# SimFlowCFD/RapidCFD-dev

Measured on AMD Instinct MI355X. Metric: PCG iterations/s + HBM GB/s on 10M-cell lduMatrix at 1/2/4/8 MI355X, higher is better.
Workload: dtype f64

## Files before the change

### __graft_entry__.py

```python
from __future__ import annotations

import importlib.util
import os
import subprocess
import sys

ROOT = os.path.dirname(os.path.abspath(__file__))
PKG_DIR = os.path.join(ROOT, "rapidcfd-dev_amd")
PKG_NAME = "rapidcfd_dev_amd"
HIPCC_FLAGS = ["--offload-arch=gfx950", "-O3", "-std=c++17", "-ffp-contract=off", "-fPIC", "-shared", "-pthread"]


def load_package():
    if PKG_NAME in sys.modules:
        return sys.modules[PKG_NAME]
    spec = importlib.util.spec_from_file_location(
        PKG_NAME, os.path.join(PKG_DIR, "__init__.py"), submodule_search_locations=[PKG_DIR])
    mod = importlib.util.module_from_spec(spec)
    sys.modules[PKG_NAME] = mod
    spec.loader.exec_module(mod)
    return mod


def _stale(target, sources):
    if not os.path.exists(target):
        return True
    t = os.path.getmtime(target)
    return any(os.path.getmtime(s) > t for s in sources)


def build() -> None:
    csrc = os.path.join(PKG_DIR, "csrc")
    srcs = [os.path.join(csrc, f) for f in ("engine.hip", "tiling.cpp", "gamg.cpp")]
    deps = srcs + [os.path.join(csrc, f) for f in ("kernels.hip.hpp", "tiling.hpp", "host_parallel.hpp", "gamg.hpp", "gamg_engine.inc", "assembly.inc", "limited_grad.inc", "comm.inc", "peer.inc", "multi.inc", "multi_pipe.inc", "persist.inc", "pcg_fused.inc", "host_tables.hpp", "host_match.hpp", "switches.hpp")] + [os.path.join(ROOT, "include", "mi_ldu.h")]
    so = os.path.join(PKG_DIR, "librapidcfd_amd.so")
    if _stale(so, deps):
        hipcc = os.environ.get("HIPCC", "/opt/rocm/bin/hipcc")
        subprocess.check_call([hipcc, *HIPCC_FLAGS, *srcs, "-o", so])
    foam = os.path.join(PKG_DIR, "foam")
    hipcc = os.environ.get("HIPCC", "/opt/rocm/bin/hipcc")
    libfoam = os.path.join(PKG_DIR, "libmiFoam.so")
    if _stale(libfoam, [os.path.join(foam, f) for f in ("miFoam.C", "miFoam.H", "polyMesh.C", "polyMesh.H", "solution.C", "solution.H")] + [so]):
        subprocess.check_call([hipcc, "--offload-arch=gfx950", "-O2", "-std=c++17", "-fPIC", "-shared", "-x", "hip",
                               os.path.join(foam, "miFoam.C"), os.path.join(foam, "polyMesh.C"), os.path.join(foam, "solution.C"), "-o", libfoam, "-L" + PKG_DIR,
                               "-lrapidcfd_amd", "-Wl,-rpath,$ORIGIN"])
    for name in ("pEqnFoam", "pEqnFoamPar", "polyMeshFoam", "polyMeshFoamPar", "icoFoam", "scalarTransportFoam"):
        app = os.path.join(PKG_DIR, name)
        if _stale(app, [os.path.join(foam, name + ".C"), libfoam]):
            subprocess.check_call(["g++", "-O2", "-std=c++17", os.path.join(foam, name + ".C"), "-o", app, "-L" + PKG_DIR,
                                   "-lmiFoam", "-lrapidcfd_amd", "-Wl,-rpath,$ORIGIN"])
    demo = os.path.join(ROOT, "examples", "c_abi_demo")
    if _stale(demo, [demo + ".c", so, os.path.join(ROOT, "include", "mi_ldu.h")]):
        subprocess.check_call(["gcc", "-std=c99", "-O2", "-Wall", "-Wextra", demo + ".c", "-I" + os.path.join(ROOT, "include"), "-I/opt/rocm/include",
                               "-D__HIP_PLATFORM_AMD__", "-L" + PKG_DIR, "-lrapidcfd_amd", "-L/opt/rocm/lib", "-lamdhip64",
                               "-Wl,-rpath,$ORIGIN/../rapidcfd-dev_amd", "-Wl,-rpath,/opt/rocm/lib", "-o", demo])
    sys.path.insert(0, ROOT)
    from oracle import oracle as _oracle
    _oracle.build()
    if os.path.isdir("/root/reference"):
        subprocess.check_call(["make", "-s", "-C", os.path.join(ROOT, "oracle"), "dropin"])
    pkg = load_package()
    pkg.engine.lib()


def smoke() -> None:
    import numpy as np
    import torch

    build()
    pkg = load_package()
    from oracle import oracle as orc
    eng = pkg.engine
    assert torch.cuda.is_available(), "smoke() needs a GPU"
    dev = torch.device("cuda:0")
    case = pkg.synthetic.box_case(24, 20, 16)
    ctx = eng.Context(0, torch.cuda.current_stream().cuda_stream)
    addr = eng.Addressing(ctx, case.n_cells, case.lower_addr, case.upper_addr)
    mat = eng.Matrix(addr)
    t = lambda a: torch.from_numpy(np.ascontiguousarray(a)).to(dev)
    mat.set_coeffs(t(case.diag), t(case.upper), None)
    psi = torch.zeros(case.n_cells, dtype=torch.float64, device=dev)
    perf = mat.pcg(psi, t(case.source), "diagonal", tolerance=1e-8, maxIter=500)
    ref_psi, ref = orc.System([case]).pcg(np.zeros(case.n_cells), case.source, "diagonal", tolerance=1e-8, maxIter=500)
    assert perf["nIterations"] == ref["nIterations"], (perf["nIterations"], ref["nIterations"])
    h, hr = perf["history"], ref["history"]
    rel = np.max(np.abs(h - hr)) / hr[0]
    assert rel < 1e-10, rel
    err = np.max(np.abs(psi.cpu().numpy() - ref_psi)) / np.max(np.abs(ref_psi))
    assert err < 1e-10, err
    print(f"smoke ok: PCG {perf['nIterations']} iterations, residual history rel diff {rel:.2e}, psi rel diff {err:.2e}")


if __name__ == "__main__":
    build()
    print("build ok")
```

### include/mi_ldu.h

```cpp
#ifndef MI_LDU_H
#define MI_LDU_H

#include <stdint.h>

#ifdef __cplusplus
extern "C" {
#endif

typedef struct mi_ctx_s *mi_ctx_t;
typedef struct mi_addr_s *mi_addr_t;
typedef struct mi_matrix_s *mi_matrix_t;
typedef struct mi_gamg_s *mi_gamg_t;
typedef struct mi_patch_s *mi_patch_t;
typedef struct mi_comm_s *mi_comm_t;

enum {
    MI_OK = 0,
    MI_ERR_ARG = -1,
    MI_ERR_DEVICE = -2,
    MI_ERR_ALLOC = -3,
    MI_ERR_STATE = -4,
    MI_ERR_LIMIT = -5,
    MI_ERR_UNSUPPORTED = -6
};

enum { MI_PRECOND_NONE = 0, MI_PRECOND_DIAGONAL = 1, MI_PRECOND_AINV = 2 };

typedef struct {
    double initialResidual;
    double finalResidual;
    double normFactor;
    int32_t nIterations;
    int32_t converged;
    int32_t singular;
    int32_t reserved;
} mi_solver_perf;

typedef struct {
    double tolerance;
    double relTol;
    int32_t maxIter;
    int32_t minIter;
} mi_solver_controls;

int mi_ctx_create(int device, void *hip_stream, mi_ctx_t *out);
int mi_ctx_destroy(mi_ctx_t ctx);
int mi_ctx_synchronize(mi_ctx_t ctx);
int mi_ctx_set_option(mi_ctx_t ctx, const char *name, int32_t value);
#define MI_STAT_PERSIST_PCG 0
#define MI_STAT_PERSIST_DPCG 1
#define MI_STAT_BARRIER_LITMUS 2
#define MI_STAT_GAMG_GRAPH_ATTACHED 3
#define MI_STAT_PCG_FUSED_RP 4
#define MI_STAT_PCG_GRAPH 5
#define MI_STAT_PBICG_MULTI 6
#define MI_STAT_PBICG_DEVICE 7
#define MI_STAT_PBICG_HOST_STEPPED 8
#define MI_STAT_PBICGSTAB_DEVICE 9
#define MI_STAT_PBICGSTAB_HOST_STEPPED 10
#define MI_STAT_PBICGSTAB_MID_EXIT 11
int mi_ctx_stat(mi_ctx_t ctx, int32_t which, int64_t *out);
const char *mi_last_error(void);
int mi_device_available(void);

int mi_addr_create(mi_ctx_t ctx, int32_t n_cells, int32_t n_faces,
                   const int32_t *lower_addr_host, const int32_t *upper_addr_host,
                   int32_t n_patches, const int32_t *patch_sizes,
                   const int32_t *const *patch_face_cells_host, mi_addr_t *out);
int mi_addr_create_coupled(mi_ctx_t ctx, int32_t n_cells, int32_t n_faces,
                           const int32_t *lower_addr_host, const int32_t *upper_addr_host,
                           int32_t n_patches, const int32_t *patch_sizes,
                           const int32_t *const *patch_face_cells_host,
                           const int32_t *const *patch_nbr_cells_host, mi_addr_t *out);
int mi_addr_set_ami_patch(mi_addr_t addr, int32_t patch, int32_t nbr_patch, const int32_t *start_host_or_null,
                          const int32_t *address_host_or_null, const double *weights_host_or_null,
                          const uint8_t *low_weight_host_or_null);
int mi_addr_set_ami_patch_remote(mi_addr_t addr, int32_t patch, int32_t transport_patch, int32_t n_partner_faces,
                                 const int32_t *start_host, const int32_t *address_host, const double *weights_host,
                                 const uint8_t *low_weight_host_or_null);
int mi_addr_set_ami_patch_remote_multi(mi_addr_t addr, int32_t patch, int32_t n_transports, const int32_t *transport_patches_host,
                                       const int32_t *n_partner_faces_host, const int32_t *start_host, const int32_t *address_host,
                                       const double *weights_host, const uint8_t *low_weight_host_or_null);
int mi_addr_set_ami_face_areas(mi_addr_t addr, int32_t patch, const double *mag_sf_host);
int mi_addr_create_ordered(mi_ctx_t ctx, int32_t n_cells, int32_t n_faces, const int32_t *lower_host, const int32_t *upper_host,
                           int32_t n_patches, const int32_t *patch_sizes, const int32_t *const *patch_face_cells_host,
                           const int32_t *const *patch_nbr_cells_host_or_null, int32_t n_tiles, const int32_t *tile_cell_start_host_or_null,
                           mi_addr_t *out);
int mi_addr_create_adopted(mi_ctx_t ctx, int32_t n_cells, int32_t n_faces, const int32_t *lower_host, const int32_t *upper_host,
                           int32_t n_patches, const int32_t *patch_sizes, const int32_t *const *patch_face_cells_host,
                           const int32_t *const *patch_nbr_cells_host_or_null, int32_t *cell_new_to_old_out, int32_t *face_new_to_old_out,
                           uint8_t *face_flipped_out, int32_t *lower_out, int32_t *upper_out, mi_addr_t *out);
int mi_layout_adopt_host(int32_t n_cells, int32_t n_faces, const int32_t *lower_host, const int32_t *upper_host, int32_t n_patches,
                         const int32_t *patch_sizes, const int32_t *const *patch_face_cells_host, const int32_t *const *patch_nbr_cells_host_or_null,
                         int32_t *cell_new_to_old_out, int32_t *face_new_to_old_out, uint8_t *face_flipped_out, int32_t *lower_out,
                         int32_t *upper_out, int32_t *n_tiles_out);
int mi_addr_tile_starts(mi_addr_t addr, int32_t *tile_cell_start_out_host);
int mi_addr_is_ordered(mi_addr_t addr);
int mi_addr_destroy(mi_addr_t addr);
int32_t mi_addr_n_cells(mi_addr_t addr);
int32_t mi_addr_n_faces(mi_addr_t addr);
int32_t mi_addr_n_tiles(mi_addr_t addr);
int32_t mi_addr_n_ext(mi_addr_t addr);
int mi_addr_cell_perm(mi_addr_t addr, int32_t *engine_to_caller_host);
int mi_addr_stats(mi_addr_t addr, int64_t stats[8]);

int mi_matrix_create(mi_addr_t addr, mi_matrix_t *out);
mi_addr_t mi_matrix_addr(mi_matrix_t m);
int mi_matrix_destroy(mi_matrix_t m);
int mi_matrix_set_coeffs(mi_matrix_t m, const double *diag_dev, const double *upper_dev,
                         const double *lower_dev);
int mi_matrix_set_interface_coeffs(mi_matrix_t m, int32_t patch, const double *bou_coeffs_dev,
                                   const double *int_coeffs_dev);
int mi_matrix_set_patch_transform(mi_matrix_t m, int32_t patch, double factor);

int mi_halo_pack_engine(mi_addr_t addr, const double *x_engine_dev, double *send_dev);
int mi_addr_patch_offsets(mi_addr_t addr, int32_t *offsets_host );

int mi_vec_to_engine(mi_addr_t addr, const double *x_caller_dev, double *x_engine_dev);
int mi_vec_from_engine(mi_addr_t addr, const double *x_engine_dev, double *x_caller_dev);

int mi_amul(mi_matrix_t m, const double *psi_dev, double *Apsi_dev);
int mi_tmul(mi_matrix_t m, const double *psi_dev, double *Tpsi_dev);
int mi_sumA(mi_matrix_t m, double *sumA_dev);
int mi_residual(mi_matrix_t m, const double *psi_dev, const double *source_dev, double *rA_dev);
int mi_H(mi_matrix_t m, const double *psi_dev, double *H_dev);
int mi_H1(mi_matrix_t m, double *H1_dev);
int mi_faceH(mi_matrix_t m, const double *psi_dev, double *faceH_dev);
int mi_matrix_set_ext(mi_matrix_t m, const double *ext_values_dev);

int mi_amul_engine(mi_matrix_t m, const double *psi_e, double *Apsi_e, int which);
int mi_tmul_engine(mi_matrix_t m, const double *psi_e, double *Tpsi_e, int which);

int mi_precondition_engine(mi_matrix_t m, int kind, int transpose, const double *rA_e, double *wA_e);
int mi_residual_engine(mi_matrix_t m, const double *psi_e, const double *source_e, double *rA_e);
int mi_jacobi_smooth_engine(mi_matrix_t m, double omega, double *psi_e, const double *source_e, int32_t n_sweeps);
int mi_norm_factor_engine(mi_matrix_t m, const double *psi_e, const double *source_e, const double *Apsi_e, double *out_host);

int mi_precondition(mi_matrix_t m, int kind, int transpose, const double *rA_dev, double *wA_dev);

int mi_jacobi_smooth(mi_matrix_t m, double omega, double *psi_dev, const double *source_dev,
                     int32_t n_sweeps);

int mi_sum(mi_ctx_t ctx, const double *a_dev, int64_t n, double *out_host);
int mi_sum_prod(mi_ctx_t ctx, const double *a_dev, const double *b_dev, int64_t n, double *out_host);
int mi_sum_mag(mi_ctx_t ctx, const double *a_dev, int64_t n, double *out_host);
int mi_norm_factor(mi_matrix_t m, const double *psi_dev, const double *source_dev,
                   const double *Apsi_dev, double *out_host);

int mi_pcg_solve(mi_matrix_t m, double *psi_dev, const double *source_dev,
                 const mi_solver_controls *controls, int precond,
                 mi_solver_perf *perf_out, double *residual_history_host, int32_t history_len);
int mi_pcg_begin(mi_matrix_t m, const double *psi0_dev, const double *source_dev,
                 const mi_solver_controls *controls, int precond, int32_t history_len);
int mi_pcg_iterate(mi_matrix_t m, int32_t n_iters, float *amul_ms_sum);
int mi_pcg_iterate_sampled(mi_matrix_t m, int32_t n_iters, int32_t event_stride, float *amul_ms_sum);
int mi_pcg_end(mi_matrix_t m, double *psi_out_dev, mi_solver_perf *perf_out,
               double *residual_history_host, int32_t history_len);

typedef struct {
    double tolerance, relTol;
    int32_t maxIter, minIter;
    int32_t nPreSweeps, preSweepsLevelMultiplier, maxPreSweeps;
    int32_t nPostSweeps, postSweepsLevelMultiplier, maxPostSweeps;
    int32_t nFinestSweeps, scaleCorrection;
    double omega;
    int32_t directSolveCoarsest;
    int32_t reserved;
} mi_gamg_controls;
int mi_gamg_create(mi_addr_t fine_addr, const double *face_weights_host, int32_t n_cells_in_coarsest_level,
                   int32_t merge_levels, int forward_init, mi_gamg_t *out);
int mi_gamg_create_dummy(mi_addr_t fine_addr, int32_t n_levels, mi_gamg_t *out);
int mi_gamg_create_coupled(mi_addr_t fine_addr, const double *face_weights_host,
                           int32_t n_cells_in_coarsest_level, int32_t merge_levels, int forward_init, mi_comm_t reduce_or_null,
                           mi_comm_t halo_or_null, const int32_t *patch_rank,
                           const int32_t *patch_nbr_patch_or_null, mi_gamg_t *out);
int mi_gamg_destroy(mi_gamg_t g);
int32_t mi_gamg_n_levels(mi_gamg_t g);
int mi_gamg_forward_out(mi_gamg_t g);
int mi_gamg_level_sizes(mi_gamg_t g, int32_t level, int32_t out4[4]);
int mi_gamg_solve(mi_gamg_t g, mi_matrix_t m, double *psi_dev, const double *source_dev,
                  const mi_gamg_controls *controls, mi_solver_perf *perf_out,
                  double *residual_history_host, int32_t history_len);
int mi_gamg_restrict(mi_gamg_t g, int32_t level, const double *fine_dev, double *coarse_dev);
int mi_gamg_prolong(mi_gamg_t g, int32_t level, const double *coarse_dev, double *fine_dev);
int mi_gamg_update(mi_gamg_t g, mi_matrix_t m);
int mi_gamg_level_matrix(mi_gamg_t g, int32_t level, mi_matrix_t *level_matrix_out);
int mi_gamg_scale(mi_matrix_t m, double *field_dev, double *Acf_dev, const double *source_dev);
int mi_gamg_solve_coarsest(mi_gamg_t g, const double *source_dev, double *corr_dev);
int mi_gamg_level_coeffs(mi_gamg_t g, mi_matrix_t m, int32_t level, double *diag_out_dev,
                         double *upper_out_dev, double *lower_out_dev);

int mi_row_face_op(mi_addr_t addr, int kind, const double *lower_dev, const double *upper_dev, double *inout_dev);
int mi_fvm_laplacian(mi_addr_t addr, const double *delta_coeffs_dev, const double *gamma_magsf_dev,
                     double *upper_out_dev, double *diag_out_dev);
int mi_fvm_div(mi_addr_t addr, const double *weights_dev, const double *face_flux_dev,
               double *lower_out_dev, double *upper_out_dev, double *diag_out_dev);
int mi_surface_integrate(mi_addr_t addr, const double *ssf_dev, const double *vol_dev_or_null, double *ivf_dev);
int mi_face_interpolate(mi_addr_t addr, const double *lambda_dev, const double *phi_dev, double *sf_dev);
int mi_fvm_ddt_euler(mi_ctx_t ctx, int64_t n, double r_delta_t, double rho, const double *vol_dev,
                     const double *psi_old_dev, double *diag_out_dev, double *source_out_dev);
int mi_upwind_weights(mi_ctx_t ctx, int64_t n_faces, const double *face_flux_dev, double *weights_out_dev);
int mi_limited_linear_weights(mi_addr_t addr, double k, const double *cd_weights_dev, const double *face_flux_dev,
                              const double *phi_dev, const double *gradx_dev, const double *grady_dev,
                              const double *gradz_dev, const double *cx_dev, const double *cy_dev,
                              const double *cz_dev, double *weights_out_dev, double *limiter_out_dev_or_null);
enum { MI_LIM_LIMITED_LINEAR, MI_LIM_VAN_LEER, MI_LIM_MUSCL, MI_LIM_MINMOD, MI_LIM_SUPERBEE, MI_LIM_UMIST,
       MI_LIM_VAN_ALBADA, MI_LIM_OSPRE, MI_LIM_QUICK, MI_LIM_LIMITED_CUBIC, MI_LIM_GAMMA, MI_LIM_SFCD };
typedef struct mi_limiter {
    int32_t kind;
    int32_t vector_form;
    int32_t bounded;
    double k, lower, upper;
} mi_limiter;
// ... 193 lines not shown
```

### rapidcfd-dev_amd/csrc/engine.hip

```cpp
#include <hip/hip_ext.h>
#include "../../include/mi_ldu.h"
#include "kernels.hip.hpp"
#include "tiling.hpp"
#include "host_parallel.hpp"
#include "switches.hpp"

#include <algorithm>
#include <atomic>
#include <cstdio>
#include <cstdlib>
#include <cstring>
#include <condition_variable>
#include <functional>
#include <map>
#include <set>
#include <mutex>
#include <string>
#include <thread>
#include <vector>

using namespace mi;
constexpr int HALO_NV = 6;

namespace {

thread_local std::string g_err;
int fail(int code, const std::string& msg) { g_err = msg; return code; }

#define HIPCHK(expr)                                                                          \
    do {                                                                                      \
        hipError_t e__ = (expr);                                                              \
        if (e__ != hipSuccess)                                                                \
            return fail(MI_ERR_DEVICE, std::string(#expr) + ": " + hipGetErrorString(e__));   \
    } while (0)
#define MICHK(expr) do { int r__ = (expr); if (r__ != MI_OK) return r__; } while (0)

template <class T>
struct DevBuf {
    T* p = nullptr;
    size_t n = 0;
    DevBuf() = default;
    DevBuf(const DevBuf&) = delete;
    DevBuf& operator=(const DevBuf&) = delete;
    ~DevBuf() { release(); }
    void release() { if (p) { (void)hipFree(p); p = nullptr; n = 0; } }
    int alloc(size_t count)
    {
        if (count == n && p) return MI_OK;
        release();
        if (hipMalloc((void**)&p, (count ? count : 1) * sizeof(T)) != hipSuccess) { p = nullptr; return fail(MI_ERR_ALLOC, "hipMalloc failed"); }
        n = count;
        return MI_OK;
    }
    template <class A>
    int upload(const std::vector<T, A>& v, hipStream_t s)
    {
        MICHK(alloc(v.size()));
        if (!v.empty()) HIPCHK(hipMemcpyAsync(p, v.data(), v.size() * sizeof(T), hipMemcpyHostToDevice, s));
        return MI_OK;
    }
};

}

struct mi_ctx_s {
    int device = 0;
    hipStream_t stream = nullptr;
    bool ownStream = false;
    DevBuf<double> partial;
    DevBuf<double> scalars;
    DevBuf<PcgState> state;
    PcgState* hostState = nullptr;
    double* hostScal = nullptr;
    hipEvent_t ev0 = nullptr, ev1 = nullptr;
    hipStream_t sideStream = nullptr;
    hipEvent_t evSideGo = nullptr, evSideDone = nullptr;
    int nCU = 0;
    bool keepSlotTables = false;
    int tileFlags = 0, attachEvents = 0, persist = 0, xcdRows = 0, deferPsi = 0, fusePerm = 0, pairAT = 0, fusePrologue = 0, multiPipe = 0, winDirect = 0, gamgGraphAttached = 0;
    int pcgPersist = 0, pcgFuseRP = 0, pcgFuseTest = 0, persistGrid = 0, persistShared = 0, fuseFinal = 0, amulBS = 0, pcgBatch = 0, pcgGraph = 0, pbicgHostStepped = 0;
    int gamgDeviceInvert = 0, gamgAlwaysAgglomerate = 0, gamgGraph = 0, gamgFuse = 0;
    int64_t stats[12] = {};
    int persistCoop = -1;
    uint64_t faultEpoch = 0;
    struct mi_matrix_s* session = nullptr;
    std::set<const void*> ldsAttrSet;
    std::map<std::pair<const void*, size_t>, int> occCache;
};

struct CtxSwitch { Switch id; int mi_ctx_s::*member; };
static constexpr CtxSwitch CTX_SWITCHES[] = {
    {SW_TILE_FLAGS, &mi_ctx_s::tileFlags}, {SW_EVENT_ATTACH, &mi_ctx_s::attachEvents}, {SW_TILE_PERSIST, &mi_ctx_s::persist}, {SW_XCD_ROWS, &mi_ctx_s::xcdRows},
    {SW_PCG_DEFER_PSI, &mi_ctx_s::deferPsi}, {SW_FUSE_PERM, &mi_ctx_s::fusePerm}, {SW_PBICG_PAIR, &mi_ctx_s::pairAT}, {SW_FUSE_PROLOGUE, &mi_ctx_s::fusePrologue},
    {SW_MULTI_PIPE, &mi_ctx_s::multiPipe}, {SW_WIN_DIRECT, &mi_ctx_s::winDirect}, {SW_GAMG_GRAPH_ATTACHED, &mi_ctx_s::gamgGraphAttached}, {SW_PCG_PERSIST, &mi_ctx_s::pcgPersist},
    {SW_PCG_FUSE_RP, &mi_ctx_s::pcgFuseRP}, {SW_PCG_FUSE_TEST, &mi_ctx_s::pcgFuseTest}, {SW_PERSIST_GRID, &mi_ctx_s::persistGrid}, {SW_PERSIST_SHARED, &mi_ctx_s::persistShared},
    {SW_PCG_FUSE_FINAL, &mi_ctx_s::fuseFinal}, {SW_AMUL_BS, &mi_ctx_s::amulBS}, {SW_PCG_BATCH, &mi_ctx_s::pcgBatch}, {SW_PCG_GRAPH, &mi_ctx_s::pcgGraph},
    {SW_PBICG_HOST_STEPPED, &mi_ctx_s::pbicgHostStepped}, {SW_GAMG_DEVICE_INVERT, &mi_ctx_s::gamgDeviceInvert}, {SW_GAMG_ALWAYS_AGGLOMERATE, &mi_ctx_s::gamgAlwaysAgglomerate},
    {SW_GAMG_GRAPH, &mi_ctx_s::gamgGraph}, {SW_GAMG_FUSE, &mi_ctx_s::gamgFuse},
};
constexpr bool ctx_switches_match_table()
{
    for (int s = 0; s < SW_COUNT; ++s) {
        int n = 0;
        for (const CtxSwitch& e : CTX_SWITCHES) n += e.id == s;
        if (n != ((sw::table[s].when & sw::CTX) ? 1 : 0)) return false;
    }
    return true;
}
static_assert(ctx_switches_match_table(), "CTX_SWITCHES: exactly one entry for every sw::CTX row of switches.hpp");
static void ctx_store(mi_ctx_s* c, const CtxSwitch& s, int value) { c->*s.member = s.id == SW_PCG_FUSE_RP ? (value != 0 ? -1 : 0) : value; }

struct mi_addr_s {
    mi_ctx_s* ctx = nullptr;
    TileLayout L;
    DevBuf<int32_t> e2c, c2e, tileCellStart, tileSlotStart, tileIfaceSlot0, tileHaloStart, haloCell, tileSliceStart, sliceEntryStart;
    DevBuf<uint32_t> entries, entries16;
    DevBuf<int32_t> sliceEntryStart16, tileSbStart;
    DevBuf<uint16_t> slotBase;
    bool compact = false;
    DevBuf<int32_t> slotFace, extSlot, interiorTiles, boundaryTiles, patchFaceCellsE, faceSlot, lowerAddr, upperAddr;
    DevBuf<int32_t> ownerStartC, losortStartC, losortC;
    DevBuf<uint32_t> row16; DevBuf<uint16_t> losort16; DevBuf<int32_t> rowEsc, rowEscStart;
    struct RowPlan { bool tiles = false; int bs = 256, blocks = 0, maxFaces = 0, capForced = 0; } rowPlan[2];
    DevBuf<double> relaxD0, relaxSumOff;
    DevBuf<uint8_t> setMask; DevBuf<double> setVal;
    Table<int32_t> lowerHost, upperHost;
    int32_t nInterior = 0, nBoundary = 0, nLocalPatches = 0;
    Table<char> patchIsLocal;
    DevBuf<int32_t> ifaceNbrCaller;
    DevBuf<int32_t> haloSrc;
    Table<Table<int32_t>> patchFaceCellsHost, patchNbrCellsHost;
    int64_t nEntries = 0, nHaloTot = 0;
    struct AmiPatch {
        int32_t patch = 0, nbrPatch = 0, n = 0, extOff = 0;
        Table<int32_t> transports, partCount;
        int32_t transport = -1, nPartner = 0;
        DevBuf<int32_t> start, cellE, ownE; DevBuf<double> w; bool hasLow = false;
        Table<int32_t> hStart, hAddr; Table<double> hW, hMagSf;
    };
    Table<AmiPatch*> ami;
    bool amiRemote = false;
    ~mi_addr_s() { for (AmiPatch* q : ami) delete q; }
    bool identity = false;
    const int32_t* perm() const { return identity ? nullptr : e2c.p; }
};

struct mi_dpcg_s { double *psi = nullptr, *src = nullptr, *pA = nullptr, *wA = nullptr, *rA = nullptr, *scal = nullptr, *send = nullptr; int precond = 0; };

enum WorkVec : size_t {
    WV_OP_X = 0, WV_OP_Y = 1, WV_OP_B = 2,
    WV_NF_APSI = 0, WV_NF_SUMA = 1, WV_NF_SRC = 2, WV_NF_PSI = 3,
    WV_PSI = 3, WV_SRC = 4, WV_PA = 5, WV_WA = 6, WV_RA = 7,
    WV_PT = 8, WV_WT = 9, WV_RT = 10,
    WV_STAB_YA = 6, WV_STAB_AYA = 8, WV_STAB_SA = 9, WV_STAB_ZA = 10, WV_STAB_TA = 11, WV_STAB_RA0 = 12,
    WV_STAB_RES1 = 13,
    WV_SMOOTH_PSI2 = 8, WV_BENCH_ZERO = 14, WV_MULTI = 16, WV_MULTI_STRIDE = 11
};

struct mi_matrix_s {
    mi_addr_s* addr = nullptr;
    mi_dpcg_s dp;
    DevBuf<double> diagE, upE, lowE, rD, sumAE;
    bool asym = false, bound = false, rDValid = false, sumAValid = false;
    Table<double> patchFactor;
    uint64_t epoch = 0;
    Table<DevBuf<double>*> work;
    DevBuf<double> hist, tilePartial;
    DevBuf<PcgState> mstate; DevBuf<double> mpartial, mhist, mtilePartial; PcgState* mhostState = nullptr;
    DevBuf<double> persistScratch;
    uint64_t persistFaultEpoch = 0;
    DevBuf<double> persistZ;
    int histLen = 0;
    int pcgIt = 0, pcgPrecond = MI_PRECOND_DIAGONAL;
    bool pcgActive = false;
    bool pcgPReady = false;
    DevBuf<unsigned int> fusedBar;
    unsigned int fusedGen = 0;
    Table<hipEvent_t> evPool;
    hipGraphExec_t pcgGraph = nullptr;
    struct { int precond = -1, batch = 0, histLen = 0; const void* hist = nullptr; const void* psi = nullptr; } pcgGraphKey;
    bool gateDone = false;
    double *proY2 = nullptr, *proY3 = nullptr;
    const double *callerX = nullptr, *callerB = nullptr; double* callerY = nullptr;
    hipEvent_t kevStart = nullptr, kevStop = nullptr;
    struct mi_dpcg_comm_s* dpc = nullptr;
    DevBuf<double> sendBuf, dscal;
    ~mi_matrix_s();
    int vec(size_t k, double** out)
    {
        while (work.size() <= k) work.push_back(new DevBuf<double>());
        const size_t need = (size_t)addr->L.nCells + (size_t)addr->L.nExt;
        if (work[k]->n != need) {
            MICHK(work[k]->alloc(need));
            HIPCHK(hipMemsetAsync(work[k]->p, 0, need * sizeof(double), addr->ctx->stream));
        }
        *out = work[k]->p;
        return MI_OK;
    }
    struct Slot { size_t k; double** out; };
    int vecs(std::initializer_list<Slot> slots) { for (const Slot& v : slots) MICHK(vec(v.k, v.out)); return MI_OK; }
};

static int solver_entry(const char* fn, const mi_matrix_s* m, bool args_ok, bool check_session = true)
{
    if (!m || !args_ok) return fail(MI_ERR_ARG, std::string(fn) + ": bad argument");
    if (!m->bound) return fail(MI_ERR_STATE, "matrix coefficients not bound");
    if (check_session && m->addr->ctx->session) return fail(MI_ERR_STATE, std::string(fn) + ": a PCG session (mi_pcg_begin) is active on this context; call mi_pcg_end first");
    return MI_OK;
}

bool comm_remote(const mi_matrix_s* m);
bool comm_attached(const mi_matrix_s* m);
bool comm_any_ami(const mi_matrix_s* m);
bool comm_any_factor(const mi_matrix_s* m);
bool comm_any_compact(const mi_matrix_s* m);
bool matrix_has_factor(const mi_matrix_s* m);
void comm_inherit_factor_flag(mi_matrix_s* level, const mi_matrix_s* fine);
int64_t comm_n_global(const mi_matrix_s* m);
int comm_exchange_start(mi_matrix_s* m, const double* send, double* vec);
int comm_exchange_wait(mi_matrix_s* m);
int comm_allreduce(mi_matrix_s* m, double* dev, size_t n);
bool peer_halo_ready(const mi_matrix_s* m);
int peer_exchange_push(mi_matrix_s* m, const double* x);
int peer_exchange_pull(mi_matrix_s* m, double* x);
int peer_exchange_push_n(mi_matrix_s* m, int nv, const double* const* xs);
int peer_exchange_pull_n(mi_matrix_s* m, int nv, double* const* xs);
bool peer_win_direct(mi_matrix_s* m);
int peer_check(mi_matrix_s* m);
int dpcg_flush_if_fused(mi_matrix_s* m);
bool peer_reduce_ready(const mi_matrix_s* m);
int peer_globalize(mi_matrix_s* m, int n, double* const* P);
int pcg_solve_attached(mi_matrix_s* m, double* psi_io, const double* source, const mi_solver_controls* ctl, int precond,
                       mi_solver_perf* perf, double* hist_host, int32_t hist_len);

extern "C" const char* mi_last_error(void) { return g_err.c_str(); }

extern "C" int mi_device_available(void)
{
    int n = 0;
    if (hipGetDeviceCount(&n) != hipSuccess || n <= 0) return 0;
    hipDeviceProp_t prop;
    if (hipGetDeviceProperties(&prop, 0) != hipSuccess) return 0;
    return strncmp(prop.gcnArchName, "gfx950", 6) == 0 ? 1 : 0;
}

extern "C" int mi_ctx_create(int device, void* hip_stream, mi_ctx_t* out)
{
    if (!out) return fail(MI_ERR_ARG, "out is NULL");
    int n = 0;
    const hipError_t e0 = hipGetDeviceCount(&n);
    if (e0 != hipSuccess || n <= 0)
        return fail(MI_ERR_DEVICE, std::string("no HIP device visible: the engine has no CPU fallback (hipGetDeviceCount: ") + hipGetErrorString(e0) + ", " + std::to_string(n) + " devices)");
    if (device < 0 || device >= n) return fail(MI_ERR_ARG, "device index out of range");
    HIPCHK(hipSetDevice(device));
    hipDeviceProp_t prop;
    HIPCHK(hipGetDeviceProperties(&prop, device));
    if (strncmp(prop.gcnArchName, "gfx950", 6) != 0)
        return fail(MI_ERR_DEVICE, std::string("engine is built for gfx950 only, found ") + prop.gcnArchName);
    mi_ctx_s* c = new mi_ctx_s();
    c->device = device;
    if (hip_stream) c->stream = (hipStream_t)hip_stream;
    else { if (hipStreamCreate(&c->stream) != hipSuccess) { delete c; return fail(MI_ERR_DEVICE, "hipStreamCreate failed"); } c->ownStream = true; }
    int r = c->partial.alloc(4 * RG);
    if (r == MI_OK) r = c->scalars.alloc(16);
    if (r == MI_OK) r = c->state.alloc(1);
    if (r != MI_OK) { delete c; return r; }
    if (hipHostMalloc((void**)&c->hostState, sizeof(PcgState)) != hipSuccess ||
        hipHostMalloc((void**)&c->hostScal, 16 * sizeof(double)) != hipSuccess ||
        hipEventCreate(&c->ev0) != hipSuccess || hipEventCreate(&c->ev1) != hipSuccess) {
        delete c; return fail(MI_ERR_DEVICE, "pinned host / event allocation failed");
    }
    { hipDeviceProp_t pr; if (hipGetDeviceProperties(&pr, device) == hipSuccess) c->nCU = pr.multiProcessorCount; }
    for (const CtxSwitch& s : CTX_SWITCHES) ctx_store(c, s, sw::get(s.id));
    if (c->pcgBatch < 1) c->pcgBatch = 1;
    if (c->amulBS != 256 && c->amulBS != 512 && c->amulBS != 1024) c->amulBS = 0;
    *out = c;
    return MI_OK;
}

extern "C" int mi_ctx_destroy(mi_ctx_t c)
{
    if (!c) return MI_OK;
    (void)hipSetDevice(c->device);
    (void)hipStreamSynchronize(c->stream);
    if (c->hostState) (void)hipHostFree(c->hostState);
    if (c->hostScal) (void)hipHostFree(c->hostScal);
    if (c->ev0) (void)hipEventDestroy(c->ev0);
    if (c->ev1) (void)hipEventDestroy(c->ev1);
    if (c->sideStream) { (void)hipStreamSynchronize(c->sideStream); (void)hipStreamDestroy(c->sideStream); }
    if (c->evSideGo) (void)hipEventDestroy(c->evSideGo);
    if (c->evSideDone) (void)hipEventDestroy(c->evSideDone);
    if (c->ownStream) (void)hipStreamDestroy(c->stream);
    delete c;
    return MI_OK;
}

extern "C" int mi_ctx_synchronize(mi_ctx_t c)
{
    if (!c) return fail(MI_ERR_ARG, "ctx is NULL");
    HIPCHK(hipStreamSynchronize(c->stream));
    return MI_OK;
}

extern "C" int mi_ctx_set_option(mi_ctx_t c, const char* name, int32_t value)
{
    if (!c || !name) return fail(MI_ERR_ARG, "mi_ctx_set_option: bad argument");
    for (const CtxSwitch& s : CTX_SWITCHES)
        if (sw::table[s.id].option && strcmp(name, sw::table[s.id].option) == 0) { ctx_store(c, s, value); return MI_OK; }
    return fail(MI_ERR_ARG, "mi_ctx_set_option: unknown option");
}

extern "C" int mi_ctx_stat(mi_ctx_t c, int32_t which, int64_t* out)
{
    if (!c || !out || which < 0 || which >= (int32_t)(sizeof(c->stats) / sizeof(c->stats[0]))) return fail(MI_ERR_ARG, "mi_ctx_stat: bad argument");
    *out = c->stats[which];
    return MI_OK;
}

static int32_t tile_reorder() { return sw::get(SW_TILE_REORDER); }
static TileParams addr_tile_params(mi_ctx_t ctx, int32_t n_cells, bool coarse, bool ordered, int32_t n_tiles, const int32_t* tile_cell_start)
{
    TileParams prm;
    prm.tileCells = sw::get(SW_TILE_CELLS);
    if (prm.tileCells <= 0) {
        int target = 1024;
        if (coarse && sw::get(SW_SMALL_TILES)) target = (int)(((int64_t)n_cells / std::max(1, ctx->nCU) + 63) / 64 * 64);
        prm.tileCells = std::min(1024, std::max(128, target));
    }
    prm.slotCap = sw::get(SW_TILE_SLOTS);
    prm.reorder = tile_reorder();
// ... 284 lines not shown
    if (r != MI_OK) { delete q; return r; }
    HIPCHK(hipStreamSynchronize(s));
    a->ami.push_back(q);
    a->patchIsLocal[(size_t)patch] = 2;
    a->nLocalPatches++;
    a->amiRemote = true;
    return MI_OK;
}
extern "C" int mi_addr_set_ami_patch_remote_multi(mi_addr_t a, int32_t patch, int32_t n_transports, const int32_t* transport_patches, const int32_t* n_partner_faces,
                                                  const int32_t* start, const int32_t* address, const double* weights, const uint8_t* low_weight)
{
    if (!a || patch < 0 || patch >= a->L.nPatches || n_transports < 1 || !transport_patches || !n_partner_faces || !start || !address || !weights)
        return fail(MI_ERR_ARG, "mi_addr_set_ami_patch_remote_multi: bad argument");
    const int32_t n = (int32_t)a->patchFaceCellsHost[(size_t)patch].size();
    Table<int32_t> tr(transport_patches, transport_patches + n_transports), cnt(n_partner_faces, n_partner_faces + n_transports), off((size_t)n_transports + 1, 0);
    for (int32_t q = 0; q < n_transports; ++q) { if (cnt[(size_t)q] < 0) return fail(MI_ERR_ARG, "mi_addr_set_ami_patch_remote_multi: negative partner face count"); off[(size_t)q + 1] = off[(size_t)q] + cnt[(size_t)q]; }
    for (int32_t i = 0; i < n; ++i) if (start[i + 1] < start[i]) return fail(MI_ERR_ARG, "mi_addr_set_ami_patch_remote_multi: start must be non-decreasing");
    const int32_t na = n > 0 || start ? start[n] : 0;
    Table<int32_t> slot((size_t)na), face((size_t)na);
    for (int32_t k = 0; k < na; ++k) {
        if (address[k] < 0 || address[k] >= off[(size_t)n_transports]) return fail(MI_ERR_ARG, "mi_addr_set_ami_patch_remote_multi: address outside the partner pieces");
        int32_t q = 0;
        while (address[k] >= off[(size_t)q + 1]) ++q;
        slot[(size_t)k] = q; face[(size_t)k] = address[k] - off[(size_t)q];
    }
    return ami_remote_impl(a, patch, tr, cnt, start, slot.data(), face.data(), address, weights, low_weight);
}
extern "C" int mi_addr_set_ami_patch_remote(mi_addr_t a, int32_t patch, int32_t transport_patch, int32_t n_partner_faces, const int32_t* start,
                                            const int32_t* address, const double* weights, const uint8_t* low_weight)
{
    return mi_addr_set_ami_patch_remote_multi(a, patch, 1, &transport_patch, &n_partner_faces, start, address, weights, low_weight);
}

extern "C" int mi_addr_set_ami_face_areas(mi_addr_t a, int32_t patch, const double* mag_sf)
{
    if (!a || !mag_sf) return fail(MI_ERR_ARG, "mi_addr_set_ami_face_areas: bad argument");
    for (mi_addr_s::AmiPatch* q : a->ami) if (q->patch == patch) { q->hMagSf.assign(mag_sf, mag_sf + q->n); return MI_OK; }
    return fail(MI_ERR_ARG, "mi_addr_set_ami_face_areas: not a cyclicAMI patch");
}

extern "C" int mi_matrix_set_patch_transform(mi_matrix_t m, int32_t patch, double factor)
{
    if (!m || patch < 0 || patch >= m->addr->L.nPatches) return fail(MI_ERR_ARG, "mi_matrix_set_patch_transform: bad argument");
    if (m->addr->patchIsLocal[(size_t)patch] == 1 && factor != 1.0)
        return fail(MI_ERR_UNSUPPORTED, "mi_matrix_set_patch_transform: a transformed cyclic patch is declared through mi_addr_set_ami_patch (one-to-one, unit weights)");
    if (comm_attached(m) && factor != 1.0 && !comm_any_factor(m))
        return fail(MI_ERR_STATE, "mi_matrix_set_patch_transform: the first transformed patch of a decomposed case is declared BEFORE mi_matrix_attach_comm (the ranks agree on the solver pipeline there)");
    if (m->patchFactor.empty()) m->patchFactor.assign((size_t)m->addr->L.nPatches, 1.0);
    if (m->patchFactor[(size_t)patch] != factor) ++m->epoch;
    m->patchFactor[(size_t)patch] = factor;
    return MI_OK;
}
extern "C" int32_t mi_addr_n_cells(mi_addr_t a) { return a ? a->L.nCells : 0; }
extern "C" int32_t mi_addr_n_faces(mi_addr_t a) { return a ? a->L.nFaces : 0; }
extern "C" int32_t mi_addr_n_tiles(mi_addr_t a) { return a ? a->L.nTiles : 0; }
extern "C" int32_t mi_addr_n_ext(mi_addr_t a) { return a ? a->L.nExt : 0; }

extern "C" int mi_addr_cell_perm(mi_addr_t a, int32_t* e2c_host)
{
    if (!a || !e2c_host) return fail(MI_ERR_ARG, "mi_addr_cell_perm: bad argument");
    memcpy(e2c_host, a->L.e2c.data(), sizeof(int32_t) * (size_t)a->L.nCells);
    return MI_OK;
}

extern "C" int mi_addr_patch_offsets(mi_addr_t a, int32_t* off)
{
    if (!a || !off) return fail(MI_ERR_ARG, "mi_addr_patch_offsets: bad argument");
    memcpy(off, a->L.patchOffset.data(), sizeof(int32_t) * a->L.patchOffset.size());
    return MI_OK;
}

static size_t lds_bytes(const TileLayout& L, bool asym, bool ainv, int32_t* offLow, int32_t* offX, int32_t* offRD, int32_t* offSB = nullptr)
{
    const int32_t slots = (L.maxSlots + 3) & ~1;
    const int32_t xlen = ((L.maxCells + 63) & ~63) + L.maxHalo + 2;
    int32_t off = slots;
    *offLow = off; if (asym) off += slots;
    *offX = off; off += (xlen + 1) & ~1;
    *offRD = off; if (ainv) off += (xlen + 1) & ~1;
    if (offSB) { *offSB = off; if (L.compact) off += (L.maxCells + L.maxHalo + 1 + 3) / 4 + 1; }
    return (size_t)off * sizeof(double);
}

extern "C" int mi_addr_stats(mi_addr_t a, int64_t st[8])
{
    if (!a || !st) return fail(MI_ERR_ARG, "mi_addr_stats: bad argument");
    int32_t o1, o2, o3;
    st[0] = a->L.nTiles; st[1] = a->L.totalSlots; st[2] = a->nEntries; st[3] = a->nHaloTot;
    st[4] = a->L.maxCells; st[5] = a->L.maxSlots; st[6] = a->L.maxHalo;
    int32_t o4;
    st[7] = (int64_t)lds_bytes(a->L, false, false, &o1, &o2, &o3, &o4);
    return MI_OK;
}

static uint64_t next_epoch() { static std::atomic<uint64_t> e{0}; return ++e; }
extern "C" mi_addr_t mi_matrix_addr(mi_matrix_t m) { return m ? m->addr : nullptr; }
extern "C" int mi_matrix_create(mi_addr_t a, mi_matrix_t* out)
{
    if (!a || !out) return fail(MI_ERR_ARG, "mi_matrix_create: bad argument");
    HIPCHK(hipSetDevice(a->ctx->device));
    mi_matrix_s* m = new mi_matrix_s();
    m->addr = a;
    int r = m->diagE.alloc((size_t)a->L.nCells);
    if (r == MI_OK) r = m->upE.alloc((size_t)a->L.totalSlots);
    if (r != MI_OK) { delete m; return r; }
    if (hipMemsetAsync(m->upE.p, 0, sizeof(double) * (size_t)a->L.totalSlots, a->ctx->stream) != hipSuccess) { delete m; return fail(MI_ERR_DEVICE, "memset failed"); }
    *out = m;
    return MI_OK;
}

extern "C" int mi_matrix_destroy(mi_matrix_t m)
{
    if (m) { (void)hipSetDevice(m->addr->ctx->device); (void)hipStreamSynchronize(m->addr->ctx->stream); delete m; }
    return MI_OK;
}

extern "C" int mi_matrix_set_coeffs(mi_matrix_t m, const double* diag, const double* upper, const double* lower)
{
    if (!m || !diag || (!upper && m->addr->L.nFaces > 0)) return fail(MI_ERR_ARG, "mi_matrix_set_coeffs: bad argument");
    mi_addr_s* a = m->addr;
    hipStream_t s = a->ctx->stream;
    HIPCHK(hipSetDevice(a->ctx->device));
    const bool asym = (lower != nullptr);
    if (asym && m->lowE.n != (size_t)a->L.totalSlots) {
        MICHK(m->lowE.alloc((size_t)a->L.totalSlots));
        HIPCHK(hipMemcpyAsync(m->lowE.p, m->upE.p, sizeof(double) * (size_t)a->L.totalSlots, hipMemcpyDeviceToDevice, s));
    }
    m->asym = asym;
    k_gather_perm<<<RG, RB, 0, s>>>(diag, a->perm(), m->diagE.p, a->L.nCells);
    k_fill_slots<<<2048, 256, 0, s>>>(upper, lower, a->slotFace.p, m->upE.p, asym ? m->lowE.p : nullptr, a->L.totalSlots);
    HIPCHK(hipGetLastError());
    m->bound = true;
    m->rDValid = false; m->sumAValid = false;
    m->epoch = next_epoch();
    return MI_OK;
}

extern "C" int mi_matrix_set_interface_coeffs(mi_matrix_t m, int32_t patch, const double* bou, const double* inte)
{
    if (!m || !bou || patch < 0 || patch >= m->addr->L.nPatches) return fail(MI_ERR_ARG, "mi_matrix_set_interface_coeffs: bad argument");
    mi_addr_s* a = m->addr;
    HIPCHK(hipSetDevice(a->ctx->device));
    const int32_t off = a->L.patchOffset[patch], n = a->L.patchOffset[(size_t)patch + 1] - off;
    if (n == 0) return MI_OK;
    k_fill_iface<<<(n + 255) / 256, 256, 0, a->ctx->stream>>>(bou, inte, a->extSlot.p + off, m->upE.p, m->asym ? m->lowE.p : nullptr, n);
    HIPCHK(hipGetLastError());
    m->sumAValid = false;
    m->epoch = next_epoch();
    return MI_OK;
}

namespace {

template <int OP, bool ASYM, bool TRANS, bool C16>
int launch_tile_bs(mi_matrix_s* m, const TileArgs& args, int nTiles, size_t lds)
{
    hipStream_t s = m->addr->ctx->stream;
    int bs = m->addr->ctx->amulBS;
    if (bs == 0) bs = (lds > 53 * 1024) ? 1024 : (m->addr->L.maxCells <= 256 ? 256 : 512);
    if (nTiles <= 0) return MI_OK;
#define MI_LAUNCH(BS)                                                                                                   \
    {                                                                                                                   \
        mi_ctx_s* cx = m->addr->ctx;                                                                                    \
        const void* fn = (const void*)tile_kernel<OP, ASYM, TRANS, BS, C16>;                                            \
        if (!cx->ldsAttrSet.count(fn)) {           \
            HIPCHK(hipFuncSetAttribute(fn, hipFuncAttributeMaxDynamicSharedMemorySize, 159 * 1024));                    \
            cx->ldsAttrSet.insert(fn);                                                                                  \
        }                                                                                                               \
        int grid = nTiles;                                                                                              \
        if (cx->persist) {                                                                                              \
            int& occ = cx->occCache[std::make_pair(fn, lds)];                                                           \
            if (occ == 0) {                                                                                             \
                int nb = 0;                                                                                             \
                HIPCHK(hipOccupancyMaxActiveBlocksPerMultiprocessor(&nb, fn, BS, lds));                                 \
                occ = nb > 0 ? nb : 1;                                                                                  \
            }                                                                                                           \
            const int slots = ((occ * cx->nCU * cx->persist) / 8) * 8;                                                  \
            if (slots >= 8 && nTiles > 2 * slots) grid = slots;                                                         \
        }                                                                                                               \
        if (m->kevStart)            \
            hipExtLaunchKernelGGL((tile_kernel<OP, ASYM, TRANS, BS, C16>), dim3(grid), dim3(BS), (uint32_t)lds, s, m->kevStart, m->kevStop, 0, args); \
        else                                                                                                            \
        tile_kernel<OP, ASYM, TRANS, BS, C16><<<grid, BS, lds, s>>>(args);                                                   \
    }
    if (bs == 1024) MI_LAUNCH(1024)
    else if (bs == 512) MI_LAUNCH(512)
    else MI_LAUNCH(256)
#undef MI_LAUNCH
    HIPCHK(hipGetLastError());
    return MI_OK;
}

template <int OP>
int launch_tile_win(mi_matrix_s* m, bool trans, const double* x, const double* b, const double* rD, double* y,
                    double omega, double* dotPartial, double* dotPartial2);

template <int OP>
int launch_tile(mi_matrix_s* m, bool trans, const double* x, const double* b, const double* rD, double* y,
                double omega, int which, double* dotPartial = nullptr, double* dotPartial2 = nullptr)
{
    mi_addr_s* a = m->addr;
    if (!m->bound) return fail(MI_ERR_STATE, "matrix coefficients not bound (mi_matrix_set_coeffs)");
    TileArgs t;
    t.tileCellStart = a->tileCellStart.p; t.tileSlotStart = a->tileSlotStart.p; t.tileIfaceSlot0 = a->tileIfaceSlot0.p; t.tileHaloStart = a->tileHaloStart.p;
    t.haloCell = a->haloCell.p; t.tileSliceStart = a->tileSliceStart.p; t.sliceEntryStart = a->sliceEntryStart.p;
    t.entries = a->entries.p; t.entries16 = a->entries16.p; t.sliceEntryStart16 = a->sliceEntryStart16.p; t.slotBase = reinterpret_cast<const uint32_t*>(a->slotBase.p); t.tileSbStart = a->tileSbStart.p;
    t.diag = m->diagE.p; t.up = m->upE.p; t.low = m->lowE.p;
    t.x = x; t.b = b; t.rD = rD; t.y = y; t.omega = omega; t.dotPartial = dotPartial; t.dotPartial2 = dotPartial2; t.flags = a->ctx->tileFlags;
    if (OP == OP_PROLOGUE) { t.y2 = m->proY2; t.y3 = m->proY3; }

    const size_t lds = lds_bytes(a->L, m->asym, OP == OP_AINV, &t.offLow, &t.offX, &t.offRD, &t.offSB);
    if (lds > 159 * 1024) return fail(MI_ERR_LIMIT, "tile needs more than 159 KiB of LDS");
    int nTiles = a->L.nTiles;
    t.tileList = nullptr;
    if (which == 1) { t.tileList = a->interiorTiles.p; nTiles = a->nInterior; }
    else if (which == 2) { t.tileList = a->boundaryTiles.p; nTiles = a->nBoundary; }
    t.nPos = nTiles;
    t.done = m->gateDone ? &a->ctx->state.p->done : nullptr;
    if (m->callerY) {
        if constexpr (OP == OP_AMUL || OP == OP_RESIDUAL || OP == OP_H || OP == OP_SUMA || OP == OP_H1) {
            t.perm = a->e2c.p; t.haloSrc = a->haloSrc.p; t.xExt = x ? x + a->L.nCells : nullptr;
            t.x = m->callerX; t.b = m->callerB; t.y = m->callerY;
            mi_ctx_s* cx = a->ctx;
            hipStream_t s = cx->stream;
            const bool big = lds > 53 * 1024;
#define MI_LAUNCH_PERM(ASYM, TRANS)                                                                                      \
            {                                                                                                           \
                const void* fn = big ? (const void*)tile_kernel_perm<OP, ASYM, TRANS, 1024> : (const void*)tile_kernel_perm<OP, ASYM, TRANS, 512>; \
                if (!cx->ldsAttrSet.count(fn)) { HIPCHK(hipFuncSetAttribute(fn, hipFuncAttributeMaxDynamicSharedMemorySize, 159 * 1024)); cx->ldsAttrSet.insert(fn); } \
                if (big) tile_kernel_perm<OP, ASYM, TRANS, 1024><<<nTiles, 1024, lds, s>>>(t);                           \
                else tile_kernel_perm<OP, ASYM, TRANS, 512><<<nTiles, 512, lds, s>>>(t);                                 \
            }
            if (nTiles > 0) {
                if (m->asym) { if (trans) MI_LAUNCH_PERM(true, true) else MI_LAUNCH_PERM(true, false) }
                else MI_LAUNCH_PERM(false, false)
            }
#undef MI_LAUNCH_PERM
            HIPCHK(hipGetLastError());
            return MI_OK;
        } else return fail(MI_ERR_STATE, "caller-order tile launch of an operator without a caller-order form");
    }
    if (a->compact) {
        if (m->asym) {
            if (trans) return launch_tile_bs<OP, true, true, true>(m, t, nTiles, lds);
            return launch_tile_bs<OP, true, false, true>(m, t, nTiles, lds);
        }
        return launch_tile_bs<OP, false, false, true>(m, t, nTiles, lds);
    }
    if (m->asym) {
        if (trans) return launch_tile_bs<OP, true, true, false>(m, t, nTiles, lds);
        return launch_tile_bs<OP, true, false, false>(m, t, nTiles, lds);
    }
    return launch_tile_bs<OP, false, false, false>(m, t, nTiles, lds);
}

struct FxArgs {
    const int32_t* map = nullptr; const double* coarse = nullptr; double* out = nullptr;
    const double *field = nullptr, *acf = nullptr, *src = nullptr, *scal = nullptr, *add = nullptr;
    unsigned int* foldCounter = nullptr; double* foldOut = nullptr;
};
inline bool tile_fx_usable(const mi_matrix_s* m) { return m->bound && !m->addr->compact && m->addr->L.nExt == 0 && m->addr->ami.empty() && !m->callerY && !m->gateDone; }
template <int OP, int XMODE>
int launch_tile_fx(mi_matrix_s* m, const FxArgs& fx, const double* b, double* y, double omega, double* dotPartial = nullptr, double* dotPartial2 = nullptr)
{
    mi_addr_s* a = m->addr;
    if (!tile_fx_usable(m)) return fail(MI_ERR_STATE, "launch_tile_fx: matrix not eligible");
    TileArgs t;
    t.tileCellStart = a->tileCellStart.p; t.tileSlotStart = a->tileSlotStart.p; t.tileIfaceSlot0 = a->tileIfaceSlot0.p; t.tileHaloStart = a->tileHaloStart.p;
    t.haloCell = a->haloCell.p; t.tileSliceStart = a->tileSliceStart.p; t.sliceEntryStart = a->sliceEntryStart.p;
    t.entries = a->entries.p; t.entries16 = nullptr; t.sliceEntryStart16 = nullptr; t.slotBase = nullptr; t.tileSbStart = nullptr;
    t.diag = m->diagE.p; t.up = m->upE.p; t.low = m->lowE.p;
    t.x = nullptr; t.b = b; t.rD = nullptr; t.y = y; t.omega = omega; t.dotPartial = dotPartial; t.dotPartial2 = dotPartial2; t.flags = a->ctx->tileFlags;
    t.fxMap = fx.map; t.fxCoarse = fx.coarse; t.fxOut = fx.out; t.fxField = fx.field; t.fxAcf = fx.acf; t.fxSrc = fx.src; t.fxScal = fx.scal; t.fxAdd = fx.add;
    t.foldCounter = fx.foldCounter; t.foldOut = fx.foldOut;
    size_t lds = lds_bytes(a->L, m->asym, false, &t.offLow, &t.offX, &t.offRD, &t.offSB);
    if (lds > 159 * 1024) return fail(MI_ERR_LIMIT, "tile needs more than 159 KiB of LDS");
    if (fx.foldOut) lds = std::max(lds, (size_t)(2 * RG + 2 * (RB / 64) + 2) * sizeof(double));
    const int nTiles = a->L.nTiles;
    t.tileList = nullptr; t.nPos = nTiles; t.done = nullptr;
    if (nTiles <= 0) return MI_OK;
    mi_ctx_s* cx = a->ctx;
    hipStream_t s = cx->stream;
    int bs = cx->amulBS;
    if (bs == 0) bs = (lds > 53 * 1024) ? 1024 : (a->L.maxCells <= 256 ? 256 : 512);
#define MI_LAUNCH_FX(ASYM, BS)                                                                                           \
    {                                                                                                                   \
        const void* fn = (const void*)tile_kernel_fx<OP, ASYM, BS, XMODE>;                                              \
        if (!cx->ldsAttrSet.count(fn)) { HIPCHK(hipFuncSetAttribute(fn, hipFuncAttributeMaxDynamicSharedMemorySize, 159 * 1024)); cx->ldsAttrSet.insert(fn); } \
        tile_kernel_fx<OP, ASYM, BS, XMODE><<<nTiles, BS, lds, s>>>(t);                                                 \
    }
    if (m->asym) { if (bs == 1024) MI_LAUNCH_FX(true, 1024) else if (bs == 512) MI_LAUNCH_FX(true, 512) else MI_LAUNCH_FX(true, 256) }
    else { if (bs == 1024) MI_LAUNCH_FX(false, 1024) else if (bs == 512) MI_LAUNCH_FX(false, 512) else MI_LAUNCH_FX(false, 256) }
#undef MI_LAUNCH_FX
    HIPCHK(hipGetLastError());
    return MI_OK;
}

int ensure_rD(mi_matrix_s* m)
{
    if (m->rDValid) return MI_OK;
    mi_addr_s* a = m->addr;
    const size_t need = (size_t)a->L.nCells + (size_t)a->L.nExt;
    if (m->rD.n != need) {
        MICHK(m->rD.alloc(need));
        HIPCHK(hipMemsetAsync(m->rD.p, 0, need * sizeof(double), a->ctx->stream));
    }
    k_recip<<<RG, RB, 0, a->ctx->stream>>>(m->rD.p, m->diagE.p, a->L.nCells);
    HIPCHK(hipGetLastError());
    m->rDValid = true;
    return MI_OK;
}

bool aligned16(const void* p) { return (reinterpret_cast<uintptr_t>(p) & 15u) == 0; }
// ... 348 lines not shown
    MICHK(m->vec(WV_OP_Y, &scratch));
    double *cur = psi_e, *nxt = scratch;
    for (int sw = 0; sw < n_sweeps; ++sw) {
        if (a->L.nExt > 0 && sw > 0 && !comm_remote(m))
            HIPCHK(hipMemcpyAsync(cur + a->L.nCells, nxt + a->L.nCells, sizeof(double) * (size_t)a->L.nExt, hipMemcpyDeviceToDevice, s));
        MICHK(tile_op<OP_JACOBI>(m, false, cur, source_e, nullptr, nxt, omega));
        double* t = cur; cur = nxt; nxt = t;
    }
    if (cur != psi_e) HIPCHK(hipMemcpyAsync(psi_e, cur, sizeof(double) * (size_t)a->L.nCells, hipMemcpyDeviceToDevice, s));
    return MI_OK;
}

namespace {
int norm_factor_engine(mi_matrix_s* m, const double* psi_e, const double* src_e, const double* Apsi_e, double* sumA_scratch, double* out)
{
    mi_addr_s* a = m->addr;
    mi_ctx_s* c = a->ctx;
    hipStream_t s = c->stream;
    const int64_t n = a->L.nCells;
    MICHK(launch_tile<OP_SUMA>(m, false, nullptr, nullptr, nullptr, sumA_scratch, 0.0, 0));
    double sumPsi = 0;
    MICHK(reduce_sync_fwd(m, psi_e, &sumPsi));
    const double avg = sumPsi / (double)(comm_attached(m) ? comm_n_global(m) : n);
    k_normfactor<<<RG, RB, 0, s>>>(Apsi_e, src_e, sumA_scratch, avg, n, c->partial.p);
    k_reduce_final<<<1, RB, 0, s>>>(c->partial.p, c->scalars.p);
    HIPCHK(hipGetLastError());
    if (comm_attached(m)) MICHK(comm_allreduce(m, c->scalars.p, 1));
    HIPCHK(hipMemcpyAsync(c->hostScal, c->scalars.p, sizeof(double), hipMemcpyDeviceToHost, s));
    HIPCHK(hipStreamSynchronize(s));
    *out = c->hostScal[0] + SP_SMALL;
    return MI_OK;
}
}
extern "C" int mi_norm_factor(mi_matrix_t m, const double* psi, const double* source, const double* Apsi, double* out)
{
    MICHK(solver_entry("mi_norm_factor", m, psi && source && Apsi && out));
    mi_addr_s* a = m->addr;
    HIPCHK(hipSetDevice(a->ctx->device));
    hipStream_t s = a->ctx->stream;
    const int64_t n = a->L.nCells;
    double *ApsiE, *sumA, *srcE, *psiE;
    MICHK(m->vecs({{WV_NF_APSI, &ApsiE}, {WV_NF_SUMA, &sumA}, {WV_NF_SRC, &srcE}, {WV_NF_PSI, &psiE}}));
    k_gather_perm<<<RG, RB, 0, s>>>(Apsi, a->perm(), ApsiE, n);
    k_gather_perm<<<RG, RB, 0, s>>>(source, a->perm(), srcE, n);
    k_gather_perm<<<RG, RB, 0, s>>>(psi, a->perm(), psiE, n);
    return norm_factor_engine(m, psiE, srcE, ApsiE, sumA, out);
}
extern "C" int mi_norm_factor_engine(mi_matrix_t m, const double* psi_e, const double* source_e, const double* Apsi_e, double* out)
{
    MICHK(solver_entry("mi_norm_factor_engine", m, psi_e && source_e && Apsi_e && out));
    HIPCHK(hipSetDevice(m->addr->ctx->device));
    double* sumA;
    MICHK(m->vec(WV_NF_SUMA, &sumA));
    return norm_factor_engine(m, psi_e, source_e, Apsi_e, sumA, out);
}

namespace {

int precond_engine(mi_matrix_s* m, int kind, bool transpose, const double* r, double* w)
{
    mi_addr_s* a = m->addr;
    hipStream_t s = a->ctx->stream;
    const int64_t n = a->L.nCells;
    if (kind == MI_PRECOND_NONE) { HIPCHK(hipMemcpyAsync(w, r, sizeof(double) * (size_t)n, hipMemcpyDeviceToDevice, s)); return MI_OK; }
    MICHK(ensure_rD(m));
    if (kind == MI_PRECOND_DIAGONAL) { k_mul<<<RG, RB, 0, s>>>(w, m->rD.p, r, n); HIPCHK(hipGetLastError()); return MI_OK; }
    if (kind == MI_PRECOND_AINV) return launch_tile<OP_AINV>(m, transpose, r, nullptr, m->rD.p, w, 0.0, 0);
    return fail(MI_ERR_ARG, "unknown preconditioner kind");
}

template <int KIND>
int reduce_sync(mi_matrix_s* m, const double* a, const double* b, double* out)
{
    mi_ctx_s* c = m->addr->ctx;
    k_reduce<KIND><<<RG, RB, 0, c->stream>>>(a, b, (int64_t)m->addr->L.nCells, c->partial.p);
    k_reduce_final<<<1, RB, 0, c->stream>>>(c->partial.p, c->scalars.p);
    HIPCHK(hipGetLastError());
    if (comm_attached(m)) MICHK(comm_allreduce(m, c->scalars.p, 1));
    HIPCHK(hipMemcpyAsync(c->hostScal, c->scalars.p, sizeof(double), hipMemcpyDeviceToHost, c->stream));
    HIPCHK(hipStreamSynchronize(c->stream));
    if (comm_attached(m)) MICHK(peer_check(m));
    *out = c->hostScal[0];
    return MI_OK;
}

int reduce_sync_fwd(mi_matrix_s* m, const double* a, double* out) { return reduce_sync<RED_SUM>(m, a, nullptr, out); }

int solve_prologue(mi_matrix_s* m, const mi_solver_controls* ctl, const double* psi_e, const double* src_e,
                   double* wA, double* rA, int histLen)
{
    mi_addr_s* a = m->addr;
    mi_ctx_s* c = a->ctx;
    hipStream_t s = c->stream;
    const int64_t n = a->L.nCells;
    if (m->hist.n < (size_t)(histLen > 0 ? histLen : 1)) MICHK(m->hist.alloc((size_t)(histLen > 0 ? histLen : 1)));
    m->histLen = histLen;
    PcgState h;
    memset(&h, 0, sizeof(h));
    h.tolerance = ctl->tolerance; h.relTol = ctl->relTol; h.maxIter = ctl->maxIter; h.minIter = ctl->minIter;
    *c->hostState = h;
    HIPCHK(hipMemcpyAsync(c->state.p, c->hostState, sizeof(PcgState), hipMemcpyHostToDevice, s));
    if (c->fusePrologue) {
        const bool needSumA = !m->sumAValid;
        if (needSumA && m->sumAE.n != (size_t)n) MICHK(m->sumAE.alloc((size_t)n));
        m->proY2 = rA; m->proY3 = needSumA ? m->sumAE.p : nullptr;
        const int rc = tile_op<OP_PROLOGUE>(m, false, psi_e, src_e, nullptr, wA, 0.0);
        m->proY2 = nullptr; m->proY3 = nullptr;
        MICHK(rc);
        m->sumAValid = true;
        double* P = c->partial.p;
        k_reduce<RED_SUM><<<RG, RB, 0, s>>>(psi_e, nullptr, n, P + 2 * RG);
        if (comm_attached(m)) {
            k_reduce_final<<<1, RB, 0, s>>>(P + 2 * RG, c->scalars.p);
            MICHK(comm_allreduce(m, c->scalars.p, 1));
            k_normfactor_mag<true><<<RG, RB, 0, s>>>(wA, src_e, m->sumAE.p, c->scalars.p, (double)comm_n_global(m), n, P, P + RG);
            k_reduce_final2<<<2, RB, 0, s>>>(P, c->scalars.p + 1, P + RG, c->scalars.p + 2);
            MICHK(comm_allreduce(m, c->scalars.p + 1, 2));
            k_solve_init<true><<<1, RB, 0, s>>>(c->state.p, c->scalars.p + 1, c->scalars.p + 2, m->hist.p, histLen);
        } else {
            k_normfactor_mag<false><<<RG, RB, 0, s>>>(wA, src_e, m->sumAE.p, P + 2 * RG, (double)n, n, P, P + RG);
            k_solve_init<false><<<1, RB, 0, s>>>(c->state.p, P, P + RG, m->hist.p, histLen);
        }
        HIPCHK(hipGetLastError());
        return MI_OK;
    }
    MICHK(tile_op<OP_AMUL>(m, false, psi_e, nullptr, nullptr, wA, 0.0));
    k_sub<<<RG, RB, 0, s>>>(rA, src_e, wA, n);
    if (!m->sumAValid) {
        if (m->sumAE.n != (size_t)n) MICHK(m->sumAE.alloc((size_t)n));
        MICHK(launch_tile<OP_SUMA>(m, false, nullptr, nullptr, nullptr, m->sumAE.p, 0.0, 0));
        m->sumAValid = true;
    }
    double sumPsi = 0;
    MICHK(reduce_sync<RED_SUM>(m, psi_e, nullptr, &sumPsi));
    const double avg = sumPsi / (double)(comm_attached(m) ? comm_n_global(m) : n);
    k_normfactor<<<RG, RB, 0, s>>>(wA, src_e, m->sumAE.p, avg, n, c->partial.p);
    k_reduce<RED_MAG><<<RG, RB, 0, s>>>(rA, nullptr, n, c->partial.p + RG);
    if (comm_attached(m)) {
        k_reduce_final2<<<2, RB, 0, s>>>(c->partial.p, c->scalars.p + 1, c->partial.p + RG, c->scalars.p + 2);
        MICHK(comm_allreduce(m, c->scalars.p + 1, 2));
        k_solve_init<true><<<1, RB, 0, s>>>(c->state.p, c->scalars.p + 1, c->scalars.p + 2, m->hist.p, histLen);
    } else
    k_solve_init<false><<<1, RB, 0, s>>>(c->state.p, c->partial.p, c->partial.p + RG, m->hist.p, histLen);
    HIPCHK(hipGetLastError());
    return MI_OK;
}

int fetch_state(mi_ctx_s* c)
{
    HIPCHK(hipMemcpyAsync(c->hostState, c->state.p, sizeof(PcgState), hipMemcpyDeviceToHost, c->stream));
    HIPCHK(hipStreamSynchronize(c->stream));
    if (c->hostState->fault) {
        c->faultEpoch++;
        return fail(MI_ERR_DEVICE, "persistent PCG kernel: a workgroup never reached a grid barrier (ran out of polls); the results of this solve are not valid");
    }
    return MI_OK;
}

template <class State>
void fill_perf(const State& h, mi_solver_perf* p)
{
    p->initialResidual = h.initialResidual; p->finalResidual = h.finalResidual; p->normFactor = h.normFactor;
    p->nIterations = h.nIterations; p->converged = h.converged; p->singular = h.singular; p->reserved = 0;
}

int copy_hist(hipStream_t s, const double* hist_dev, int dev_len, double* hist_host, int len, int nIter, bool sync = true)
{
    if (!hist_host || len <= 0) return MI_OK;
    int cnt = nIter + 1; if (cnt > len) cnt = len; if (cnt > dev_len) cnt = dev_len;
    if (cnt > 0) {
        HIPCHK(hipMemcpyAsync(hist_host, hist_dev, sizeof(double) * (size_t)cnt, hipMemcpyDeviceToHost, s));
        if (sync) HIPCHK(hipStreamSynchronize(s));
    }
    return MI_OK;
}
int copy_hist(mi_matrix_s* m, double* hist_host, int len, int nIter) { return copy_hist(m->addr->ctx->stream, m->hist.p, m->histLen, hist_host, len, nIter); }

struct PcgVecs { double *psi, *src, *pA, *wA, *rA; };
struct BicgVecs : PcgVecs { double *pT, *wT, *rT; };
struct StabVecs { double *psi, *src, *pA, *yA, *rA, *AyA, *sA, *zA, *tA, *rA0; };
int work_vecs(mi_matrix_s* m, PcgVecs& v) { return m->vecs({{WV_PSI, &v.psi}, {WV_SRC, &v.src}, {WV_PA, &v.pA}, {WV_WA, &v.wA}, {WV_RA, &v.rA}}); }
int work_vecs(mi_matrix_s* m, BicgVecs& v) { MICHK(work_vecs(m, static_cast<PcgVecs&>(v))); return m->vecs({{WV_PT, &v.pT}, {WV_WT, &v.wT}, {WV_RT, &v.rT}}); }
int work_vecs(mi_matrix_s* m, StabVecs& v) { return m->vecs({{WV_PSI, &v.psi}, {WV_SRC, &v.src}, {WV_PA, &v.pA}, {WV_STAB_YA, &v.yA}, {WV_RA, &v.rA},
                                                             {WV_STAB_AYA, &v.AyA}, {WV_STAB_SA, &v.sA}, {WV_STAB_ZA, &v.zA}, {WV_STAB_TA, &v.tA}, {WV_STAB_RA0, &v.rA0}}); }
template <class Vecs>
int stage_in(mi_matrix_s* m, Vecs& v, const double* psi, const double* source)
{
    mi_addr_s* a = m->addr;
    MICHK(work_vecs(m, v));
    k_gather_perm<<<RG, RB, 0, a->ctx->stream>>>(psi, a->perm(), v.psi, a->L.nCells);
    k_gather_perm<<<RG, RB, 0, a->ctx->stream>>>(source, a->perm(), v.src, a->L.nCells);
    return MI_OK;
}

struct GateDone { mi_matrix_s* m; explicit GateDone(mi_matrix_s* mm) : m(mm) { m->gateDone = true; } ~GateDone() { m->gateDone = false; } };
int iter_limit(const mi_solver_controls* ctl) { return ctl->maxIter + (ctl->minIter > ctl->maxIter ? ctl->minIter : 0); }

template <class Enqueue, class Fetch, class Done>
int drive_batches(mi_matrix_s* m, const mi_solver_controls* ctl, const int& it, int first, Enqueue enqueue, Fetch fetch, Done done)
{
    const int batch = m->addr->ctx->pcgBatch, limit = iter_limit(ctl);
    int nb = batch < first ? batch : first;
    while (!done() && it <= limit) {
        MICHK(enqueue(nb));
        MICHK(fetch());
        MICHK(peer_check(m));
        nb = nb * 2 > batch ? batch : nb * 2;
    }
    return MI_OK;
}
template <class Enqueue>
int drive_batches(mi_matrix_s* m, const mi_solver_controls* ctl, const int& it, int first, Enqueue enqueue)
{
    mi_ctx_s* c = m->addr->ctx;
    return drive_batches(m, ctl, it, first, enqueue, [c] { return fetch_state(c); }, [c] { return c->hostState->done != 0; });
}

int finish_device(mi_matrix_s* m, const double* psi_e, double* psi_out, mi_solver_perf* perf, double* hist_host, int hist_len, int (*flush)(mi_matrix_s*) = nullptr)
{
    mi_addr_s* a = m->addr; mi_ctx_s* c = a->ctx;
    if (flush) MICHK(flush(m));
    k_scatter_perm<<<RG, RB, 0, c->stream>>>(psi_e, a->perm(), psi_out, a->L.nCells);
    HIPCHK(hipGetLastError());
    if (perf) fill_perf(*c->hostState, perf);
    MICHK(copy_hist(m, hist_host, hist_len, c->hostState->nIterations));
    HIPCHK(hipStreamSynchronize(c->stream));
    return MI_OK;
}

int globalize(mi_matrix_s* m, double* PA, double* PB = nullptr)
{
    if (!comm_attached(m)) return MI_OK;
    if (peer_reduce_ready(m)) { double* P[2] = {PA, PB}; return peer_globalize(m, PB ? 2 : 1, P); }
    mi_ctx_s* c = m->addr->ctx;
    hipStream_t s = c->stream;
    double* sc = c->scalars.p + 10;
    if (PB) k_reduce_final2<<<2, RB, 0, s>>>(PA, sc, PB, sc + 1);
    else k_reduce_final<<<1, RB, 0, s>>>(PA, sc);
    MICHK(comm_allreduce(m, sc, PB ? 2 : 1));
    k_spread_partials<<<PB ? 2 : 1, RB, 0, s>>>(sc, PA, PB);
    HIPCHK(hipGetLastError());
    return MI_OK;
}

bool pcg_fused_rp_usable(const mi_matrix_s* m, int precond);
int pcg_fused_rp_launch(mi_matrix_s* m, int it, int precond);
bool pcg_persist_usable(const mi_matrix_s* m, int precond);
int pcg_persist_enqueue(mi_matrix_s* m, int n_iters, int precond);
int pcg_enqueue(mi_matrix_s* m, int it0, int count, int precond, int evStride)
{
    mi_addr_s* a = m->addr;
    mi_ctx_s* c = a->ctx;
    hipStream_t s = c->stream;
    const int64_t n = a->L.nCells;
    PcgVecs v;
    MICHK(work_vecs(m, v));
    double *psi = v.psi, *pA = v.pA, *wA = v.wA, *rA = v.rA;
    double* P1 = c->partial.p; double* P2 = c->partial.p + RG; double* P3 = c->partial.p + 2 * RG;
    if (precond != MI_PRECOND_NONE) MICHK(ensure_rD(m));
    if (m->tilePartial.n < (size_t)a->L.nTiles) MICHK(m->tilePartial.alloc((size_t)a->L.nTiles));
    const bool fuse = c->fuseFinal && precond != MI_PRECOND_AINV;
    const int defer = (c->deferPsi && !fuse) ? 1 : 0;
    double* psiD = defer ? psi : nullptr;
    GateDone gate(m);
    bool fusedRP = it0 >= 0 && pcg_fused_rp_usable(m, precond);
    if (it0 < 0) m->pcgPReady = false;
    for (int k = 0; k < count; ++k) {
        const int it = it0 < 0 ? -1 : it0 + k;
        if (m->pcgPReady) {
        } else
        if (precond == MI_PRECOND_AINV) {
            MICHK(launch_tile<OP_AINV>(m, false, rA, nullptr, m->rD.p, wA, 0.0, 0, m->tilePartial.p));
            k_fold_partials<<<1, 1024, 0, s>>>(m->tilePartial.p, a->L.nTiles, P1);
            MICHK(globalize(m, P1));
            k_pcg_update_p<0><<<RG, RB, 0, s>>>(c->state.p, it, P1, wA, nullptr, nullptr, pA, n, nullptr, nullptr, 0, psiD);
        } else if (precond == MI_PRECOND_DIAGONAL) {
            k_pcg_update_p<1><<<RG, RB, 0, s>>>(c->state.p, it, P1, nullptr, m->rD.p, rA, pA, n, fuse ? P3 : nullptr, m->hist.p, m->histLen, psiD);
        } else {
            k_pcg_update_p<2><<<RG, RB, 0, s>>>(c->state.p, it, P1, nullptr, nullptr, rA, pA, n, fuse ? P3 : nullptr, m->hist.p, m->histLen, psiD);
        }
        const bool rec = evStride > 0 && (k % evStride) == 0;
        const size_t ev = rec ? (size_t)2 * (size_t)(k / evStride) : 0;
        if (rec) {
            while (m->evPool.size() < ev + 2) { hipEvent_t e; HIPCHK(hipEventCreate(&e)); m->evPool.push_back(e); }
            if (c->attachEvents) { m->kevStart = m->evPool[ev]; m->kevStop = m->evPool[ev + 1]; }
            else HIPCHK(hipEventRecord(m->evPool[ev], s));
        }
        const int rcA = tile_op<OP_AMUL>(m, false, pA, nullptr, nullptr, wA, 0.0, m->tilePartial.p);
        m->kevStart = nullptr; m->kevStop = nullptr;
        MICHK(rcA);
        if (rec && !c->attachEvents) HIPCHK(hipEventRecord(m->evPool[ev + 1], s));
        k_fold_partials<<<1, 1024, 0, s>>>(m->tilePartial.p, a->L.nTiles, P2);
        MICHK(globalize(m, P2));
        m->pcgPReady = false;
        if (fusedRP) {
            const int rcF = pcg_fused_rp_launch(m, it, precond);
            if (rcF == MI_OK) { m->pcgPReady = true; continue; }
            if (rcF != MI_ERR_UNSUPPORTED) return rcF;
            fusedRP = false;
        }
        if (precond == MI_PRECOND_AINV)
            k_pcg_update_psi_r<0><<<RG, RB, 0, s>>>(c->state.p, it, P2, pA, wA, nullptr, psi, rA, n, P3, P1, defer);
        else if (precond == MI_PRECOND_DIAGONAL)
            k_pcg_update_psi_r<1><<<RG, RB, 0, s>>>(c->state.p, it, P2, pA, wA, m->rD.p, psi, rA, n, P3, P1, defer);
        else
            k_pcg_update_psi_r<2><<<RG, RB, 0, s>>>(c->state.p, it, P2, pA, wA, nullptr, psi, rA, n, P3, P1, defer);
        MICHK(globalize(m, P3, precond == MI_PRECOND_AINV ? nullptr : P1));
        if (!fuse) k_pcg_final<false><<<1, RB, 0, s>>>(c->state.p, it, P3, m->hist.p, m->histLen);
    }
    if (count > 0 && fuse) k_pcg_final<false><<<1, RB, 0, s>>>(c->state.p, it0 < 0 ? -1 : it0 + count - 1, P3, m->hist.p, m->histLen);
    HIPCHK(hipGetLastError());
    return MI_OK;
}

int pcg_first_dot(mi_matrix_s* m, int precond, const PcgVecs& v)
{
    mi_ctx_s* c = m->addr->ctx;
    if (precond != MI_PRECOND_DIAGONAL && precond != MI_PRECOND_NONE) return MI_OK;
    if (precond == MI_PRECOND_DIAGONAL) MICHK(ensure_rD(m));
    if (precond == MI_PRECOND_DIAGONAL) k_pcg_precond_dot<true><<<RG, RB, 0, c->stream>>>(c->state.p, m->rD.p, v.rA, v.wA, m->addr->L.nCells, c->partial.p);
    else k_pcg_precond_dot<false><<<RG, RB, 0, c->stream>>>(c->state.p, nullptr, v.rA, v.wA, m->addr->L.nCells, c->partial.p);
    HIPCHK(hipGetLastError());
    return globalize(m, c->partial.p);
}

int pcg_flush(mi_matrix_s* m)
{
    mi_ctx_s* c = m->addr->ctx;
    if (!c->deferPsi) return MI_OK;
    double *psi, *pA;
    MICHK(m->vecs({{WV_PSI, &psi}, {WV_PA, &pA}}));
    k_pcg_flush_psi<<<RG, RB, 0, c->stream>>>(c->state.p, pA, psi, m->addr->L.nCells);
    k_pcg_flush_mark<<<1, 1, 0, c->stream>>>(c->state.p);
    HIPCHK(hipGetLastError());
    return MI_OK;
}

}

extern "C" int mi_pcg_begin(mi_matrix_t m, const double* psi0, const double* source,
                            const mi_solver_controls* ctl, int precond, int32_t history_len)
{
    if (!m || !psi0 || !source || !ctl) return fail(MI_ERR_ARG, "mi_pcg_begin: bad argument");
    if (!m->bound) return fail(MI_ERR_STATE, "matrix coefficients not bound");
    if (comm_attached(m)) return fail(MI_ERR_STATE, "mi_pcg_begin: a communicator is attached; use mi_pcg_solve or the mi_dpcg_* session");
    if (m->addr->ctx->session && m->addr->ctx->session != m)
        return fail(MI_ERR_STATE, "mi_pcg_begin: another matrix has a PCG session open on this context (one session per context: it owns the solver scratch)");
    mi_addr_s* a = m->addr;
    HIPCHK(hipSetDevice(a->ctx->device));
    PcgVecs v;
    MICHK(stage_in(m, v, psi0, source));
    MICHK(solve_prologue(m, ctl, v.psi, v.src, v.wA, v.rA, history_len));
    MICHK(pcg_first_dot(m, precond, v));
    m->pcgIt = 0; m->pcgPrecond = precond; m->pcgActive = true; m->pcgPReady = false; a->ctx->session = m;
    return MI_OK;
}

extern "C" int mi_pcg_iterate_sampled(mi_matrix_t m, int32_t n_iters, int32_t event_stride, float* amul_ms_sum);
extern "C" int mi_pcg_iterate(mi_matrix_t m, int32_t n_iters, float* amul_ms_sum)
{
    if (!m || !m->pcgActive || n_iters < 0) return fail(MI_ERR_STATE, "mi_pcg_iterate: no active PCG session");
    HIPCHK(hipSetDevice(m->addr->ctx->device));
    return mi_pcg_iterate_sampled(m, n_iters, amul_ms_sum ? 1 : 0, amul_ms_sum);
}

extern "C" int mi_pcg_iterate_sampled(mi_matrix_t m, int32_t n_iters, int32_t event_stride, float* amul_ms_sum)
{
    if (!m || !m->pcgActive || n_iters < 0 || event_stride < 0) return fail(MI_ERR_STATE, "mi_pcg_iterate: no active PCG session");
    HIPCHK(hipSetDevice(m->addr->ctx->device));
    const int stride = amul_ms_sum ? (event_stride > 0 ? event_stride : 1) : 0;
    if (!amul_ms_sum && !m->pcgPReady && pcg_persist_usable(m, m->pcgPrecond)) {
        const int rcP = pcg_persist_enqueue(m, n_iters, m->pcgPrecond);
        if (rcP != MI_ERR_UNSUPPORTED) {
            MICHK(rcP);
            m->pcgIt += n_iters;
            return MI_OK;
        }
    }
    MICHK(pcg_enqueue(m, m->pcgIt, n_iters, m->pcgPrecond, stride));
    m->pcgIt += n_iters;
    if (amul_ms_sum) {
        HIPCHK(hipStreamSynchronize(m->addr->ctx->stream));
        const int ns = (n_iters + stride - 1) / stride;
        float tot = 0;
        for (int i = 0; i < ns; ++i) { float ms = 0; HIPCHK(hipEventElapsedTime(&ms, m->evPool[(size_t)2 * i], m->evPool[(size_t)2 * i + 1])); tot += ms; }
        *amul_ms_sum = ns > 0 ? tot * ((float)n_iters / (float)ns) : 0.f;
    }
    return MI_OK;
}

extern "C" int mi_pcg_end(mi_matrix_t m, double* psi_out, mi_solver_perf* perf, double* hist_host, int32_t hist_len)
{
    if (!m || !m->pcgActive) return fail(MI_ERR_STATE, "mi_pcg_end: no active PCG session");
    mi_addr_s* a = m->addr;
    HIPCHK(hipSetDevice(a->ctx->device));
    double* psi;
    MICHK(m->vec(WV_PSI, &psi));
    MICHK(pcg_flush(m));
    if (psi_out) k_scatter_perm<<<RG, RB, 0, a->ctx->stream>>>(psi, a->perm(), psi_out, a->L.nCells);
    HIPCHK(hipGetLastError());
    MICHK(fetch_state(a->ctx));
    if (perf) fill_perf(*a->ctx->hostState, perf);
    m->pcgActive = false; a->ctx->session = nullptr;
    MICHK(copy_hist(m, hist_host, hist_len, a->ctx->hostState->nIterations));
    return MI_OK;
}

extern "C" int mi_pcg_solve(mi_matrix_t m, double* psi, const double* source, const mi_solver_controls* ctl,
                            int precond, mi_solver_perf* perf, double* hist_host, int32_t hist_len)
{
    MICHK(solver_entry("mi_pcg_solve", m, psi && source && ctl, !(m && comm_attached(m))));
    if (comm_attached(m)) return pcg_solve_attached(m, psi, source, ctl, precond, perf, hist_host, hist_len);
    MICHK(mi_pcg_begin(m, psi, source, ctl, precond, ctl->maxIter + 2));
    mi_ctx_s* c = m->addr->ctx;
    struct SessionGuard { mi_matrix_s* m; ~SessionGuard() { if (m->pcgActive) { m->pcgActive = false; m->addr->ctx->session = nullptr; } } } sessionGuard{m};
    MICHK(fetch_state(c));
    const int wantGraph = c->pcgGraph;
    const bool useGraph = !pcg_persist_usable(m, precond) && (precond == MI_PRECOND_DIAGONAL || precond == MI_PRECOND_NONE) && !c->fuseFinal &&
                          (wantGraph == 1 || (wantGraph < 0 && m->addr->L.nCells <= 4000000));
    if (useGraph && !c->hostState->done) {
        const int batch = c->pcgBatch, limit = iter_limit(ctl);
        double* psiE; MICHK(m->vec(WV_PSI, &psiE));
        auto& K = m->pcgGraphKey;
        if (!m->pcgGraph || K.precond != precond || K.batch != batch || K.histLen != m->histLen || K.hist != m->hist.p || K.psi != psiE) {
            if (m->pcgGraph) { (void)hipGraphExecDestroy(m->pcgGraph); m->pcgGraph = nullptr; }
            if (precond != MI_PRECOND_NONE) MICHK(ensure_rD(m));
            if (m->tilePartial.n < (size_t)m->addr->L.nTiles) MICHK(m->tilePartial.alloc((size_t)m->addr->L.nTiles));
            hipGraph_t g = nullptr;
            HIPCHK(hipStreamBeginCapture(c->stream, hipStreamCaptureModeThreadLocal));
            const int rcE = pcg_enqueue(m, -1, batch, precond, 0);
            const hipError_t eE = hipStreamEndCapture(c->stream, &g);
            MICHK(rcE);
            HIPCHK(eE);
            const hipError_t eI = hipGraphInstantiate(&m->pcgGraph, g, nullptr, nullptr, 0);
            (void)hipGraphDestroy(g);
            HIPCHK(eI);
            K.precond = precond; K.batch = batch; K.histLen = m->histLen; K.hist = m->hist.p; K.psi = psiE;
        }
        while (!c->hostState->done && m->pcgIt <= limit) {
            HIPCHK(hipGraphLaunch(m->pcgGraph, c->stream));
            c->stats[5] += 1;
            m->pcgIt += batch;
            MICHK(fetch_state(c));
        }
        return mi_pcg_end(m, psi, perf, hist_host, hist_len);
    }
    MICHK(drive_batches(m, ctl, m->pcgIt, 2, [m](int nb) { return mi_pcg_iterate(m, nb, nullptr); }));
    return mi_pcg_end(m, psi, perf, hist_host, hist_len);
}



extern "C" int mi_dpcg_set_buffers(mi_matrix_t m, double* psi_e, double* src_e, double* pA_e, double* wA_e, double* rA_e,
                                   double* scal8, double* send_buf, const mi_solver_controls* ctl, int precond, int32_t history_len)
{
    if (!m || !psi_e || !src_e || !pA_e || !wA_e || !rA_e || !scal8 || !ctl) return fail(MI_ERR_ARG, "mi_dpcg_set_buffers: bad argument");
    if (precond != MI_PRECOND_DIAGONAL && precond != MI_PRECOND_NONE) return fail(MI_ERR_ARG, "distributed PCG supports the diagonal / none preconditioners");
    if (!m->bound) return fail(MI_ERR_STATE, "matrix coefficients not bound");
    if (comm_any_ami(m) || comm_any_factor(m))
        return fail(MI_ERR_UNSUPPORTED, "the phase-split distributed PCG does not interpolate cyclicAMI / transformed patches: use mi_pcg_solve on the attached matrix");
    mi_ctx_s* c = m->addr->ctx;
    HIPCHK(hipSetDevice(c->device));
    m->dp.psi = psi_e; m->dp.src = src_e; m->dp.pA = pA_e; m->dp.wA = wA_e; m->dp.rA = rA_e; m->dp.scal = scal8; m->dp.send = send_buf; m->dp.precond = precond;
    const int histLen = history_len > 0 ? history_len : 1;
    if (m->hist.n < (size_t)histLen) MICHK(m->hist.alloc((size_t)histLen));
    m->histLen = history_len;
    if (m->tilePartial.n < (size_t)m->addr->L.nTiles) MICHK(m->tilePartial.alloc((size_t)m->addr->L.nTiles));
    PcgState h; memset(&h, 0, sizeof(h));
    h.tolerance = ctl->tolerance; h.relTol = ctl->relTol; h.maxIter = ctl->maxIter; h.minIter = ctl->minIter;
    *c->hostState = h;
    HIPCHK(hipMemcpyAsync(c->state.p, c->hostState, sizeof(PcgState), hipMemcpyHostToDevice, c->stream));
    if (precond == MI_PRECOND_DIAGONAL) MICHK(ensure_rD(m));
    return MI_OK;
}

extern "C" int mi_dpcg_phase(mi_matrix_t m, int phase, int32_t it, double arg)
{
    if (!m || !m->dp.psi) return fail(MI_ERR_STATE, "mi_dpcg_phase: call mi_dpcg_set_buffers first");
    mi_addr_s* a = m->addr;
    mi_ctx_s* c = a->ctx;
    HIPCHK(hipSetDevice(c->device));
    hipStream_t s = c->stream;
    const int64_t n = a->L.nCells;
    const mi_dpcg_s& B = m->dp;
    double* P = c->partial.p;
    auto finalize = [&](const double* partial, double* dst) { k_reduce_final<<<1, RB, 0, s>>>(partial, dst); };
    switch (phase) {
    case 0:
        MICHK(mi_halo_pack_engine(a, B.psi, B.send));
        break;
    case 1:
        MICHK(launch_tile<OP_AMUL>(m, false, B.psi, nullptr, nullptr, B.wA, 0.0, 0));
        k_sub<<<RG, RB, 0, s>>>(B.rA, B.src, B.wA, n);
        MICHK(launch_tile<OP_SUMA>(m, false, nullptr, nullptr, nullptr, B.pA, 0.0, 0));
        k_reduce<RED_SUM><<<RG, RB, 0, s>>>(B.psi, nullptr, n, P);
        finalize(P, B.scal + 3);
        break;
    case 2:
        k_normfactor<<<RG, RB, 0, s>>>(B.wA, B.src, B.pA, arg, n, P);
        finalize(P, B.scal + 4);
        k_reduce<RED_MAG><<<RG, RB, 0, s>>>(B.rA, nullptr, n, P + RG);
        finalize(P + RG, B.scal + 1);
        if (B.precond == MI_PRECOND_DIAGONAL) k_pcg_precond_dot<true><<<RG, RB, 0, s>>>(c->state.p, m->rD.p, B.rA, B.wA, n, P + 2 * RG);
        else k_pcg_precond_dot<false><<<RG, RB, 0, s>>>(c->state.p, nullptr, B.rA, B.wA, n, P + 2 * RG);
        finalize(P + 2 * RG, B.scal + 0);
        break;
    case 3:
        k_solve_init<true><<<1, RB, 0, s>>>(c->state.p, B.scal + 4, B.scal + 1, m->hist.p, m->histLen);
        break;
    case 10:
        if (B.precond == MI_PRECOND_DIAGONAL) k_pcg_update_p<1, true><<<RG, RB, 0, s>>>(c->state.p, it, B.scal + 0, nullptr, m->rD.p, B.rA, B.pA, n, B.scal + 1, m->hist.p, m->histLen);
        else k_pcg_update_p<2, true><<<RG, RB, 0, s>>>(c->state.p, it, B.scal + 0, nullptr, nullptr, B.rA, B.pA, n, B.scal + 1, m->hist.p, m->histLen);
        MICHK(mi_halo_pack_engine(a, B.pA, B.send));
        break;
    case 11:
        MICHK(launch_tile<OP_AMUL>(m, false, B.pA, nullptr, nullptr, B.wA, 0.0, 1, m->tilePartial.p));
        break;
    case 12:
        MICHK(launch_tile<OP_AMUL>(m, false, B.pA, nullptr, nullptr, B.wA, 0.0, 2, m->tilePartial.p + a->nInterior));
        k_fold_final<<<1, 1024, 0, s>>>(m->tilePartial.p, a->L.nTiles, B.scal + 2);
        break;
    case 13:
        if (B.precond == MI_PRECOND_DIAGONAL)
            k_pcg_update_psi_r<1, true><<<RG, RB, 0, s>>>(c->state.p, it, B.scal + 2, B.pA, B.wA, m->rD.p, B.psi, B.rA, n, P + RG, P + 2 * RG);
        else
            k_pcg_update_psi_r<2, true><<<RG, RB, 0, s>>>(c->state.p, it, B.scal + 2, B.pA, B.wA, nullptr, B.psi, B.rA, n, P + RG, P + 2 * RG);
        k_reduce_final2<<<2, RB, 0, s>>>(P + RG, B.scal + 1, P + 2 * RG, B.scal + 0);
        break;
    case 14:
        k_pcg_final<true><<<1, RB, 0, s>>>(c->state.p, it, B.scal + 1, m->hist.p, m->histLen);
        break;
    default:
        return fail(MI_ERR_ARG, "mi_dpcg_phase: unknown phase");
    }
    HIPCHK(hipGetLastError());
    return MI_OK;
}

extern "C" int mi_dpcg_status(mi_matrix_t m, mi_solver_perf* perf, int32_t* done, double* hist_host, int32_t hist_len)
{
    if (!m || !perf) return fail(MI_ERR_ARG, "mi_dpcg_status: bad argument");
    mi_ctx_s* c = m->addr->ctx;
    HIPCHK(hipSetDevice(c->device));
    MICHK(dpcg_flush_if_fused(m));
    MICHK(fetch_state(c));
    MICHK(peer_check(m));
    fill_perf(*c->hostState, perf);
    if (done) *done = c->hostState->done;
    MICHK(copy_hist(m, hist_host, hist_len, c->hostState->nIterations));
    return MI_OK;
}

namespace {
struct HostPerf {
    double initialResidual = 0, finalResidual = 0, normFactor = 0;
    int nIterations = 0, converged = 0, singular = 0;
    double tolerance, relTol; int maxIter, minIter;
    void controls(const mi_solver_controls* ctl) { tolerance = ctl->tolerance; relTol = ctl->relTol; maxIter = ctl->maxIter; minIter = ctl->minIter; }
    bool checkConvergence()
    {
        converged = (finalResidual < tolerance) || (relTol > SP_SMALL && finalResidual < relTol * initialResidual);
        return converged != 0;
    }
    bool checkSingularity(double v) { singular = (v < SP_VSMALL); return singular != 0; }
};

int finish_host(mi_matrix_s* m, const HostPerf& hp, const Table<double>& hist, double* psi_e, double* psi_out,
                mi_solver_perf* perf, double* hist_host, int hist_len)
{
    mi_addr_s* a = m->addr;
    k_scatter_perm<<<RG, RB, 0, a->ctx->stream>>>(psi_e, a->perm(), psi_out, a->L.nCells);
    HIPCHK(hipGetLastError());
    HIPCHK(hipStreamSynchronize(a->ctx->stream));
    if (perf) fill_perf(hp, perf);
    if (hist_host) for (int i = 0; i < hist_len && i < (int)hist.size(); ++i) hist_host[i] = hist[(size_t)i];
    return MI_OK;
}

int host_prologue(mi_matrix_s* m, const mi_solver_controls* ctl, const double* psi_e, const double* src_e,
                  double* wA, double* rA, HostPerf& hp, Table<double>& hist)
{
    MICHK(solve_prologue(m, ctl, psi_e, src_e, wA, rA, 1));
    MICHK(fetch_state(m->addr->ctx));
    const PcgState& h = *m->addr->ctx->hostState;
    hp.controls(ctl);
    hp.normFactor = h.normFactor; hp.initialResidual = h.initialResidual; hp.finalResidual = h.finalResidual;
    hist.clear(); hist.push_back(hp.initialResidual);
    return MI_OK;
}
int host_prologue(mi_matrix_s* m, const mi_solver_controls* ctl, const double* psi_e, const double* src_e, double* wA, double* rA, double*, HostPerf& hp, Table<double>& hist) { return host_prologue(m, ctl, psi_e, src_e, wA, rA, hp, hist); }
}

namespace {
int tile_pair(mi_matrix_s* m, bool ainv, const double* x0, const double* x1, double* y0, double* y1, const int32_t* gate, double* dotPartial, bool* fused);
int multi_exchange(mi_matrix_s* m, int nv, double* const* xs);
int bicg_enqueue(mi_matrix_s* m, int it0, int count, int precond, const BicgVecs& v)
{
    double *psi = v.psi, *pA = v.pA, *wA = v.wA, *rA = v.rA, *pT = v.pT, *wT = v.wT, *rT = v.rT;
    mi_addr_s* a = m->addr;
    mi_ctx_s* c = a->ctx;
// ... 173 lines not shown

extern "C" int mi_pbicgstab_solve(mi_matrix_t m, double* psi_io, const double* source, const mi_solver_controls* ctl,
                                  int precond, int replicate_quirk, mi_solver_perf* perf, double* hist_host, int32_t hist_len)
{
    MICHK(solver_entry("mi_pbicgstab_solve", m, psi_io && source && ctl));
    mi_addr_s* a = m->addr;
    HIPCHK(hipSetDevice(a->ctx->device));
    if (m->addr->ctx->pbicgHostStepped == 0)
        return pbicgstab_solve_device(m, psi_io, source, ctl, precond, replicate_quirk, perf, hist_host, hist_len);
    hipStream_t s = a->ctx->stream;
    const int64_t n = a->L.nCells;
    StabVecs v; double* res1;
    MICHK(stage_in(m, v, psi_io, source));
    MICHK(m->vec(WV_STAB_RES1, &res1));
    double *psi = v.psi, *src = v.src, *pA = v.pA, *yA = v.yA, *rA = v.rA, *AyA = v.AyA, *sA = v.sA, *zA = v.zA, *tA = v.tA, *rA0 = v.rA0;
    HostPerf hp; Table<double> hist;
    a->ctx->stats[10] += 1;
    MICHK(host_prologue(m, ctl, psi, src, yA, rA, hp, hist));
    if (hp.minIter > 0 || !hp.checkConvergence()) {
        HIPCHK(hipMemcpyAsync(rA0, rA, sizeof(double) * (size_t)n, hipMemcpyDeviceToDevice, s));
        double rA0rA = 0, alpha = 0, omega = 0;
        do {
            const double rA0rAold = rA0rA;
            MICHK(reduce_sync<RED_PROD>(m, rA0, rA, &rA0rA));
            if (hp.checkSingularity(fabs(rA0rA))) break;
            if (hp.nIterations == 0) {
                HIPCHK(hipMemcpyAsync(pA, rA, sizeof(double) * (size_t)n, hipMemcpyDeviceToDevice, s));
            } else {
                if (hp.checkSingularity(fabs(omega))) break;
                const double beta = (rA0rA / rA0rAold) * (alpha / omega);
                k_xpsy<<<RG, RB, 0, s>>>(res1, pA, -omega, AyA, n);
                k_xpsy<<<RG, RB, 0, s>>>(pA, rA, beta, res1, n);
            }
            MICHK(precond_engine(m, precond, false, pA, yA));
            MICHK(tile_op<OP_AMUL>(m, false, yA, nullptr, nullptr, AyA, 0.0));
            double rA0AyA = 0;
            MICHK(reduce_sync<RED_PROD>(m, rA0, AyA, &rA0AyA));
            alpha = rA0rA / rA0AyA;
            k_xpsy<<<RG, RB, 0, s>>>(sA, rA, -alpha, AyA, n);
            double sm = 0;
            MICHK(reduce_sync<RED_MAG>(m, sA, nullptr, &sm));
            hp.finalResidual = sm / hp.normFactor;
            if (hp.checkConvergence()) {
                k_xpsy<<<RG, RB, 0, s>>>(psi, psi, alpha, yA, n);
                hp.nIterations++;
                hist.push_back(hp.finalResidual);
                a->ctx->stats[11] += 1;
                return finish_host(m, hp, hist, psi, psi_io, perf, hist_host, hist_len);
            }
            MICHK(precond_engine(m, precond, false, sA, zA));
            MICHK(tile_op<OP_AMUL>(m, false, zA, nullptr, nullptr, tA, 0.0));
            double tAtA = 0, tAsA = 0;
            MICHK(reduce_sync<RED_PROD>(m, tA, tA, &tAtA));
            MICHK(reduce_sync<RED_PROD>(m, tA, sA, &tAsA));
            omega = tAsA / tAtA;
            k_xpsy<<<RG, RB, 0, s>>>(psi, psi, alpha, yA, n);
            k_xpsy<<<RG, RB, 0, s>>>(psi, psi, omega, replicate_quirk ? yA : zA, n);
            k_xpsy<<<RG, RB, 0, s>>>(rA, sA, -omega, tA, n);
            MICHK(reduce_sync<RED_MAG>(m, rA, nullptr, &sm));
            hp.finalResidual = sm / hp.normFactor;
            hist.push_back(hp.finalResidual);
        } while ((hp.nIterations++ < hp.maxIter && !hp.checkConvergence()) || hp.nIterations < hp.minIter);
    }
    return finish_host(m, hp, hist, psi, psi_io, perf, hist_host, hist_len);
}

extern "C" int mi_smooth_solve(mi_matrix_t m, double* psi_io, const double* source, const mi_solver_controls* ctl,
                               double omega, int32_t n_sweeps, mi_solver_perf* perf, double* hist_host, int32_t hist_len)
{
    MICHK(solver_entry("mi_smooth_solve", m, psi_io && source && ctl && n_sweeps != 0));
    mi_addr_s* a = m->addr;
    HIPCHK(hipSetDevice(a->ctx->device));
    PcgVecs v; double* psi2;
    MICHK(stage_in(m, v, psi_io, source));
    MICHK(m->vec(WV_SMOOTH_PSI2, &psi2));
    double *src = v.src, *rA = v.rA;
    HostPerf hp; Table<double> hist;
    hp.controls(ctl);
    double *cur = v.psi, *nxt = psi2;
    auto sweeps = [&](int cnt) -> int {
        for (int sw = 0; sw < cnt; ++sw) {
            MICHK(tile_op<OP_JACOBI>(m, false, cur, src, nullptr, nxt, omega));
            double* t = cur; cur = nxt; nxt = t;
        }
        return MI_OK;
    };
    if (n_sweeps < 0) {
        MICHK(sweeps(-n_sweeps));
        hp.nIterations -= n_sweeps;
    } else {
        MICHK(host_prologue(m, ctl, v.psi, src, v.wA, rA, hp, hist));
        if (hp.minIter > 0 || !hp.checkConvergence()) {
            do {
                MICHK(sweeps(n_sweeps));
                MICHK(tile_op<OP_RESIDUAL>(m, false, cur, src, nullptr, rA, 0.0));
                double sm = 0;
                MICHK(reduce_sync<RED_MAG>(m, rA, nullptr, &sm));
                hp.finalResidual = sm / hp.normFactor;
                hist.push_back(hp.finalResidual);
            } while (((hp.nIterations += n_sweeps) < hp.maxIter && !hp.checkConvergence()) || hp.nIterations < hp.minIter);
        }
    }
    return finish_host(m, hp, hist, cur, psi_io, perf, hist_host, hist_len);
}

extern "C" int mi_debug_occupancy(mi_matrix_t m, int32_t* blocks_per_cu, int32_t* lds_bytes_out, int32_t* block_size)
{
    if (!m || !blocks_per_cu) return fail(MI_ERR_ARG, "mi_debug_occupancy: bad argument");
    mi_addr_s* a = m->addr;
    HIPCHK(hipSetDevice(a->ctx->device));
    int32_t o1, o2, o3, o4;
    const size_t lds = lds_bytes(a->L, m->asym, false, &o1, &o2, &o3, &o4);
    const int bs = a->ctx->amulBS ? a->ctx->amulBS : ((lds > 53 * 1024) ? 1024 : (a->L.maxCells <= 256 ? 256 : 512));
    int nb = 0;
#define MI_OCC(BS) { if (a->compact) HIPCHK(hipOccupancyMaxActiveBlocksPerMultiprocessor(&nb, (const void*)tile_kernel<OP_AMUL, false, false, BS, true>, BS, lds)); \
                     else HIPCHK(hipOccupancyMaxActiveBlocksPerMultiprocessor(&nb, (const void*)tile_kernel<OP_AMUL, false, false, BS, false>, BS, lds)); }
    if (bs == 1024) MI_OCC(1024) else if (bs == 512) MI_OCC(512) else MI_OCC(256)
#undef MI_OCC
    *blocks_per_cu = nb;
    if (lds_bytes_out) *lds_bytes_out = (int32_t)lds;
    if (block_size) *block_size = bs;
    return MI_OK;
}

extern "C" int mi_bench_amul(mi_matrix_t m, int32_t reps, float* ms_out)
{
    if (!m || reps <= 0 || !ms_out) return fail(MI_ERR_ARG, "mi_bench_amul: bad argument");
    mi_ctx_s* c = m->addr->ctx;
    HIPCHK(hipSetDevice(c->device));
    double *x, *y;
    MICHK(m->vecs({{WV_PA, &x}, {WV_WA, &y}}));
    HIPCHK(hipEventRecord(c->ev0, c->stream));
    for (int i = 0; i < reps; ++i) MICHK(launch_tile<OP_AMUL>(m, false, x, nullptr, nullptr, y, 0.0, 0));
    HIPCHK(hipEventRecord(c->ev1, c->stream));
    HIPCHK(hipEventSynchronize(c->ev1));
    HIPCHK(hipEventElapsedTime(ms_out, c->ev0, c->ev1));
    return MI_OK;
}

extern "C" int mi_bench_pcg_iters(mi_matrix_t m, const double* source, int32_t iters, int precond, float* ms_out, float* amul_ms_out)
{
    if (!m || !source || iters <= 0 || !ms_out) return fail(MI_ERR_ARG, "mi_bench_pcg_iters: bad argument");
    mi_ctx_s* c = m->addr->ctx;
    HIPCHK(hipSetDevice(c->device));
    mi_solver_controls ctl; ctl.tolerance = 0; ctl.relTol = 0; ctl.maxIter = iters + 16; ctl.minIter = 0;
    double* zero;
    MICHK(m->vec(WV_BENCH_ZERO, &zero));
    MICHK(mi_pcg_begin(m, zero, source, &ctl, precond, 1));
    HIPCHK(hipEventRecord(c->ev0, c->stream));
    MICHK(pcg_enqueue(m, 0, iters, precond, 0));
    HIPCHK(hipEventRecord(c->ev1, c->stream));
    HIPCHK(hipEventSynchronize(c->ev1));
    HIPCHK(hipEventElapsedTime(ms_out, c->ev0, c->ev1));
    m->pcgActive = false; c->session = nullptr;
    if (amul_ms_out) { float t = 0; MICHK(mi_bench_amul(m, iters, &t)); *amul_ms_out = t; }
    return MI_OK;
}

extern "C" int mi_layout_build_host(int32_t n_cells, int32_t n_faces, const int32_t* lower, const int32_t* upper,
                                    int32_t n_patches, const int32_t* patch_sizes, const int32_t* const* patch_face_cells,
                                    const int32_t* const* patch_nbr_cells, int32_t tile_cells, int32_t slot_cap, void** out)
{
    if (!out) return fail(MI_ERR_ARG, "mi_layout_build_host: out is NULL");
    TileLayout* L = new TileLayout();
    TileParams prm;
    if (tile_cells > 0) prm.tileCells = tile_cells;
    if (slot_cap > 0) prm.slotCap = slot_cap;
    prm.reorder = tile_reorder();
    const std::string err = build_tile_layout(n_cells, n_faces, lower, upper, n_patches, patch_sizes, patch_face_cells, prm, *L, patch_nbr_cells);
    if (!err.empty()) { delete L; return fail(MI_ERR_LIMIT, "mi_layout_build_host: " + err); }
    *out = L;
    return MI_OK;
}

extern "C" int mi_layout_build_host_given(int32_t n_cells, int32_t n_faces, const int32_t* lower, const int32_t* upper, int32_t n_parts, const int32_t* part, void** out)
{
    if (!out || !part) return fail(MI_ERR_ARG, "mi_layout_build_host_given: bad argument");
    TileLayout* L = new TileLayout();
    TileParams prm;
    prm.givenPart = part; prm.nGivenParts = n_parts;
    const std::string err = build_tile_layout(n_cells, n_faces, lower, upper, 0, nullptr, nullptr, prm, *L, nullptr);
    if (!err.empty()) { delete L; return fail(MI_ERR_LIMIT, "mi_layout_build_host_given: " + err); }
    *out = L;
    return MI_OK;
}
extern "C" int mi_layout_inherit_tiles(int32_t n_fine, const int32_t* restrict_map, const int32_t* fine_tile_of_cell, int32_t n_fine_tiles, int32_t n_coarse,
                                       int32_t n_coarse_faces, const int32_t* c_lower, const int32_t* c_upper, int32_t cell_cap, int32_t slot_cap,
                                       int32_t* part_out, int32_t* n_parts_out)
{
    if (!restrict_map || !fine_tile_of_cell || !part_out || !n_parts_out) return fail(MI_ERR_ARG, "mi_layout_inherit_tiles: bad argument");
    Table<int32_t> part;
    int32_t nParts = 0;
    const std::string err = inherit_tiles(n_fine, restrict_map, fine_tile_of_cell, n_fine_tiles, n_coarse, n_coarse_faces, c_lower, c_upper, 0, nullptr, nullptr,
                                          cell_cap > 0 ? cell_cap : 1024, slot_cap > 0 ? slot_cap : 4094, part, nParts);
    if (!err.empty()) return fail(MI_ERR_LIMIT, "mi_layout_inherit_tiles: " + err);
    std::copy(part.begin(), part.end(), part_out);
    *n_parts_out = nParts;
    return MI_OK;
}

extern "C" int mi_layout_array(void* handle, const char* name, const void** data, int64_t* len)
{
    if (!handle || !name || !data || !len) return fail(MI_ERR_ARG, "mi_layout_array: bad argument");
    TileLayout* L = static_cast<TileLayout*>(handle);
    const std::string n(name);
#define ARR(field) if (n == #field) { *data = L->field.data(); *len = (int64_t)L->field.size(); return MI_OK; }
    ARR(e2c) ARR(c2e) ARR(tileCellStart) ARR(tileSlotStart) ARR(tileIfaceSlot0) ARR(tileHaloStart) ARR(haloCell) ARR(tileSliceStart)
    ARR(sliceEntryStart) ARR(entries) ARR(sliceEntryStart16) ARR(entries16) ARR(slotBase) ARR(tileSbStart) ARR(slotFace) ARR(extSlot) ARR(interiorTiles) ARR(boundaryTiles)
    ARR(patchOffset) ARR(patchFaceCellsE) ARR(faceSlot)
#undef ARR
    return fail(MI_ERR_ARG, "mi_layout_array: unknown array " + n);
}

extern "C" int mi_layout_free(void* handle) { delete static_cast<TileLayout*>(handle); return MI_OK; }

extern "C" int mi_event_record(mi_matrix_t m, int32_t idx)
{
    if (!m || idx < 0) return fail(MI_ERR_ARG, "mi_event_record: bad argument");
    HIPCHK(hipSetDevice(m->addr->ctx->device));
    while (m->evPool.size() <= (size_t)idx) { hipEvent_t ev; HIPCHK(hipEventCreate(&ev)); m->evPool.push_back(ev); }
    HIPCHK(hipEventRecord(m->evPool[(size_t)idx], m->addr->ctx->stream));
    return MI_OK;
}
extern "C" int mi_event_elapsed_ms(mi_matrix_t m, int32_t idx0, int32_t idx1, float* ms)
{
    if (!m || !ms || idx0 < 0 || idx1 < 0 || (size_t)idx0 >= m->evPool.size() || (size_t)idx1 >= m->evPool.size()) return fail(MI_ERR_ARG, "mi_event_elapsed_ms: bad argument");
    HIPCHK(hipEventSynchronize(m->evPool[(size_t)idx1]));
    HIPCHK(hipEventElapsedTime(ms, m->evPool[(size_t)idx0], m->evPool[(size_t)idx1]));
    return MI_OK;
}

#include "multi_pipe.inc"
#include "multi.inc"
#include "comm.inc"
#include "persist.inc"
#include "pcg_fused.inc"
#include "gamg_engine.inc"
#include "assembly.inc"
#include "limited_grad.inc"

mi_matrix_s::~mi_matrix_s()
{
    if (pcgGraph) (void)hipGraphExecDestroy(pcgGraph);
    if (mhostState) (void)hipHostFree(mhostState);
    for (auto* w : work) delete w;
    for (auto e : evPool) (void)hipEventDestroy(e);
    if (dpc) {
        if (dpc->commStream) (void)hipStreamDestroy(dpc->commStream);
        if (dpc->evPack) (void)hipEventDestroy(dpc->evPack);
        if (dpc->evHalo) (void)hipEventDestroy(dpc->evHalo);
        delete dpc->ph;
        delete dpc;
    }
}
```

### rapidcfd-dev_amd/csrc/pcg_fused.inc

```
namespace mi {

constexpr int FUSED_HR = 5;
constexpr int FUSED_PF = 3;
constexpr int FUSED_LP = 2544;
constexpr int FUSED_BAR_WORDS = BAR_LINE * (RG + 64) + RG + 64;
constexpr int FUSED_PEND_AT = BAR_LINE * (RG + 64);
constexpr long long FUSED_WAIT_POLLS = 1000;
static_assert(sw::table[SW_PCG_FUSE_POLLS].dflt == FUSED_WAIT_POLLS, "switches.hpp: the default of MI_PCG_FUSE_POLLS is FUSED_WAIT_POLLS");

struct FusedArgs {
    PcgState* st;
    int it;
    const double* partial2;
    double *partial3, *partial1;
    const double *wA, *rD;
    double *pA, *psi, *rA;
    int64_t n;
    double* hist; int histLen;
    unsigned int* bar; unsigned int gen;
    long long maxPolls;
    int testMode;
};

__device__ __forceinline__ void st_agent(double* p, double v)
{
    __hip_atomic_store(reinterpret_cast<unsigned long long*>(p), (unsigned long long)__double_as_longlong(v), __ATOMIC_RELAXED, __HIP_MEMORY_SCOPE_AGENT);
}
__device__ __forceinline__ double ld_agent(const double* p)
{
    return __longlong_as_double((long long)__hip_atomic_load(reinterpret_cast<const unsigned long long*>(p), __ATOMIC_RELAXED, __HIP_MEMORY_SCOPE_AGENT));
}
__device__ __forceinline__ double sum_partials_agent(const double* partial, double* red)
{
    double v = 0;
#pragma unroll
    for (int k = 0; k < RG / RB; ++k) v += ld_agent(partial + threadIdx.x + k * RB);
    return block_sum<RB>(v, red);
}

__device__ __forceinline__ void fused_arrive(unsigned int* bar, unsigned int target, int* flag)
{
    __builtin_amdgcn_fence(__ATOMIC_RELEASE, "workgroup");
    __builtin_amdgcn_s_waitcnt(0);
    if (threadIdx.x == 0) *flag = 1;
    __syncthreads();
    if (blockIdx.x != 0 && threadIdx.x == 0) __hip_atomic_store(&bar[blockIdx.x * BAR_LINE], target, __ATOMIC_RELAXED, __HIP_MEMORY_SCOPE_AGENT);
}
__device__ __forceinline__ bool fused_wait(unsigned int* bar, unsigned int target, long long maxPolls, int testMode, int* flag)
{
    const unsigned int b = blockIdx.x, tid = threadIdx.x;
    if (b == 0) {
        if (testMode & 2) { if (tid == 0) *flag = 0; }
        else
        for (unsigned int w = tid; w < (unsigned int)RG; w += RB) {
            if (w == 0) continue;
            long long polls = 0;
            while (__hip_atomic_load(&bar[w * BAR_LINE], __ATOMIC_RELAXED, __HIP_MEMORY_SCOPE_AGENT) != target) {
                if (++polls > maxPolls) { *flag = 0; break; }
                __builtin_amdgcn_s_sleep(1);
            }
        }
        __syncthreads();
        if (*flag != 0 && tid < 64) __hip_atomic_store(&bar[(RG + tid) * BAR_LINE], target, __ATOMIC_RELAXED, __HIP_MEMORY_SCOPE_AGENT);
    } else {
        if (tid == 0) {
            const unsigned int* line = &bar[(RG + (b & 63u)) * BAR_LINE];
            long long polls = 0;
            if ((testMode & 1) && b % 3u == 1u) *flag = 0;
            else
            while (__hip_atomic_load(line, __ATOMIC_RELAXED, __HIP_MEMORY_SCOPE_AGENT) != target) {
                if (++polls > 2 * maxPolls) { *flag = 0; break; }
                __builtin_amdgcn_s_sleep(1);
            }
        }
        __syncthreads();
    }
    __builtin_amdgcn_fence(__ATOMIC_ACQUIRE, "workgroup");
    const bool ok = *flag != 0;
    __syncthreads();
    return ok;
}

struct FusedScalars { double res, wArA, beta; bool conv, cont; };
template <bool AGENT>
__device__ __forceinline__ FusedScalars fused_scalars(const PcgState* st, int it, const double* partial3, const double* partial1, double wArAold, double* red)
{
    FusedScalars q;
    q.res = (AGENT ? sum_partials_agent(partial3, red) : sum_partials(partial3, red)) / st->normFactor;
    q.conv = sp_converged(st, q.res);
    q.cont = (it < st->maxIter && !q.conv) || (it + 1 < st->minIter);
    q.wArA = AGENT ? sum_partials_agent(partial1, red) : sum_partials(partial1, red);
    q.beta = q.wArA / wArAold;
    return q;
}
__device__ __forceinline__ void fused_close(PcgState* st, int it, double alpha, double wApA, const FusedScalars& q, double* hist, int histLen)
{
    st->alpha = alpha; st->wApA = wApA;
    st->finalResidual = q.res;
    if (it + 1 < histLen) hist[it + 1] = q.res;
    st->nIterations = it + 1;
    st->it = it + 1;
    st->converged = q.conv;
    if (q.cont) st->wArA[(it + 1) & 1] = q.wArA; else st->done = 1;
    st->pApplyItP1 = st->rItP1;
}

template <int PMODE>
__global__ __launch_bounds__(RB, 8) void k_pcg_fused_r_p(FusedArgs a)
{
    extern __shared__ double2 zLds[];
    __shared__ double red[RB / 64];
    __shared__ int flag;
    PcgState* __restrict__ st = a.st;
    if (st->done) return;
    const int it = a.it;
    const unsigned int b = blockIdx.x, tid = threadIdx.x;
    const bool lead = b == 0 && tid == 0;
    const double wApA = sum_partials(a.partial2, red);
    if (fabs(wApA) / st->normFactor < SP_VSMALL) {
        if (tid == 0) a.partial3[b] = -1.0;
        if (lead) { st->singular = 1; st->done = 1; }
        return;
    }
    const double wArAold = st->wArA[it & 1];
    const double alpha = wArAold / wApA;
    const Chunk ck = my_chunk(a.n);
    const double* __restrict__ wA = a.wA + ck.lo; const double* __restrict__ rD = a.rD + (PMODE == 1 ? ck.lo : 0);
    double* __restrict__ rA = a.rA + ck.lo; double* __restrict__ pA = a.pA + ck.lo; double* __restrict__ psi = a.psi + ck.lo;
    const int len = (int)(ck.hi - ck.lo), np = len >> 1;
    const bool oddTail = (len & 1) && tid == 0;
    double acc0 = 0, acc1 = 0, d0 = 0, d1 = 0;
    double2 zr[FUSED_HR];
    double zTail = 0.0;
    auto residual2 = [&](int i) -> double2 {
        const double2 w = ld2_stream(wA, i);
        double2 r = ld2(rA, i);
        r.x = fma(-alpha, w.x, r.x); r.y = fma(-alpha, w.y, r.y);
        st2(rA, i, r); acc0 += fabs(r.x); acc1 += fabs(r.y);
        double2 z = r;
        if (PMODE == 1) { const double2 d = ld2_rd(rD, i); z.x = d.x * r.x; z.y = d.y * r.y; }
        d0 = fma(z.x, r.x, d0); d1 = fma(z.y, r.y, d1);
        return z;
    };
#pragma unroll
    for (int k = 0; k < FUSED_HR; ++k) {
        const int q = (int)tid + k * RB;
        zr[k] = make_double2(0.0, 0.0);
        if (q < np) zr[k] = residual2(2 * q);
    }
    for (int q = (int)tid + FUSED_HR * RB; q < np; q += RB) {
        const double2 z = residual2(2 * q);
        const int l = q - FUSED_HR * RB;
        if (l < FUSED_LP) zLds[l] = z;
    }
    if (oddTail) {
        const int i = len - 1;
        const double r = fma(-alpha, wA[i], rA[i]); rA[i] = r; acc0 += fabs(r);
        zTail = (PMODE == 1) ? rD[i] * r : r;
        d0 = fma(zTail, r, d0);
    }
    const double t = block_sum<RB>(acc0 + acc1, red);
    const double u = block_sum<RB>(d0 + d1, red);
    if (tid == 0) { st_agent(a.partial3 + b, t); st_agent(a.partial1 + b, u); }
    fused_arrive(a.bar, a.gen, &flag);
    double2 pf[FUSED_PF];
#pragma unroll
    for (int k = 0; k < FUSED_PF; ++k) {
        const int q = (int)tid + k * RB;
        pf[k] = make_double2(0.0, 0.0);
        if (q < np) {
            const int i = 2 * q;
            pf[k] = ld2(pA, i);
            double2 x = ld2_stream(psi, i);
            x.x = fma(alpha, pf[k].x, x.x); x.y = fma(alpha, pf[k].y, x.y);
            st2_stream(psi, i, x);
        }
    }
    if (!fused_wait(a.bar, a.gen, a.maxPolls, a.testMode, &flag)) {
        if (tid == 0) __hip_atomic_store(&a.bar[FUSED_PEND_AT + b], 1u, __ATOMIC_RELAXED, __HIP_MEMORY_SCOPE_AGENT);
        if (lead) __hip_atomic_store(&a.bar[FUSED_PEND_AT + RG], 1u, __ATOMIC_RELAXED, __HIP_MEMORY_SCOPE_AGENT);
        return;
    }
    const FusedScalars sc = fused_scalars<true>(st, it, a.partial3, a.partial1, wArAold, red);
    const bool cont = sc.cont;
    const double beta = sc.beta;
    auto direction2 = [&](int i, double2 z) {
        const double2 p = ld2(pA, i);
        double2 x = ld2_stream(psi, i);
        x.x = fma(alpha, p.x, x.x); x.y = fma(alpha, p.y, x.y);
        st2_stream(psi, i, x);
        if (cont) st2(pA, i, make_double2(fma(beta, p.x, z.x), fma(beta, p.y, z.y)));
    };
#pragma unroll
    for (int k = 0; k < FUSED_HR; ++k) {
        const int q = (int)tid + k * RB;
        if (q < np) {
            if (k < FUSED_PF) { if (cont) st2(pA, 2 * q, make_double2(fma(beta, pf[k].x, zr[k].x), fma(beta, pf[k].y, zr[k].y))); }
            else direction2(2 * q, zr[k]);
        }
    }
    for (int q = (int)tid + FUSED_HR * RB; q < np; q += RB) {
        const int l = q - FUSED_HR * RB, i = 2 * q;
        double2 z;
        if (l < FUSED_LP) z = zLds[l];
        else { z = ld2(rA, i); if (PMODE == 1) { const double2 d = ld2_rd(rD, i); z.x = d.x * z.x; z.y = d.y * z.y; } }
        direction2(i, z);
    }
    if (oddTail) {
        const int i = len - 1;
        const double p = pA[i];
        psi[i] = fma(alpha, p, psi[i]);
        if (cont) pA[i] = fma(beta, p, zTail);
    }
    if (lead) fused_close(st, it, alpha, wApA, sc, a.hist, a.histLen);
}

template <int PMODE>
__global__ __launch_bounds__(RB) void k_pcg_fused_finish(FusedArgs a)
{
    __shared__ double red[RB / 64];
    const unsigned int b = blockIdx.x, tid = threadIdx.x;
    unsigned int* pend = a.bar + FUSED_PEND_AT;
    PcgState* __restrict__ st = a.st;
    if (b == 0 && tid == 0 && st->rItP1 >= a.it) st->pApplyItP1 = a.it;
    const bool mine = pend[b] != 0u, closing = b == 0 && pend[RG] != 0u;
    if (!mine && !closing) return;
    const int it = a.it;
    const double wApA = sum_partials(a.partial2, red);
    const double wArAold = st->wArA[it & 1];
    const double alpha = wArAold / wApA;
    const FusedScalars sc = fused_scalars<false>(st, it, a.partial3, a.partial1, wArAold, red);
    if (mine) {
        const Chunk ck = my_chunk(a.n);
        const double* __restrict__ rD = a.rD + (PMODE == 1 ? ck.lo : 0); const double* __restrict__ rA = a.rA + ck.lo;
        double* __restrict__ pA = a.pA + ck.lo; double* __restrict__ psi = a.psi + ck.lo;
        const int len = (int)(ck.hi - ck.lo), np = len >> 1;
        for (int q = (int)tid; q < np; q += RB) {
            const int i = 2 * q;
            double2 z = ld2(rA, i);
            if (PMODE == 1) { const double2 d = ld2_rd(rD, i); z.x = d.x * z.x; z.y = d.y * z.y; }
            const double2 p = ld2(pA, i);
            if (q >= FUSED_PF * RB) {
                double2 x = ld2(psi, i);
                x.x = fma(alpha, p.x, x.x); x.y = fma(alpha, p.y, x.y);
                st2(psi, i, x);
            }
            if (sc.cont) st2(pA, i, make_double2(fma(sc.beta, p.x, z.x), fma(sc.beta, p.y, z.y)));
        }
        if ((len & 1) && tid == 0) {
            const int i = len - 1;
            const double z = (PMODE == 1) ? rD[i] * rA[i] : rA[i];
            const double p = pA[i];
            psi[i] = fma(alpha, p, psi[i]);
            if (sc.cont) pA[i] = fma(sc.beta, p, z);
        }
    }
    __syncthreads();
    if (tid == 0) { pend[b] = 0u; if (closing) { fused_close(st, it, alpha, wApA, sc, a.hist, a.histLen); pend[RG] = 0u; } }
}

}

namespace {

bool pcg_fused_rp_usable(const mi_matrix_s* m, int precond)
{
    const mi_ctx_s* c = m->addr->ctx;
    return c->pcgFuseRP != 0 && !comm_attached(m) && (precond == MI_PRECOND_DIAGONAL || precond == MI_PRECOND_NONE) && !c->fuseFinal;
}

int pcg_fused_rp_launch(mi_matrix_s* m, int it, int precond)
{
    mi_addr_s* a = m->addr;
    mi_ctx_s* c = a->ctx;
    hipStream_t s = c->stream;
    const void* fn = precond == MI_PRECOND_DIAGONAL ? (const void*)k_pcg_fused_r_p<1> : (const void*)k_pcg_fused_r_p<2>;
    const size_t lds = sizeof(double2) * (size_t)FUSED_LP;
    if (c->pcgFuseRP < 0) {
        int perCU = 0, nCU = 0;
        (void)hipDeviceGetAttribute(&nCU, hipDeviceAttributeMultiprocessorCount, c->device);
        for (const void* f : {(const void*)k_pcg_fused_r_p<1>, (const void*)k_pcg_fused_r_p<2>}) {
            int q = 0;
            if (hipOccupancyMaxActiveBlocksPerMultiprocessor(&q, f, RB, lds) != hipSuccess) { (void)hipGetLastError(); q = 0; }
            perCU = (f == (const void*)k_pcg_fused_r_p<1>) ? q : std::min(perCU, q);
        }
        c->pcgFuseRP = ((int64_t)perCU * nCU >= RG) ? 1 : 0;
        if (!c->pcgFuseRP) return MI_ERR_UNSUPPORTED;
    }
    if (m->fusedBar.n < (size_t)FUSED_BAR_WORDS) {
        MICHK(m->fusedBar.alloc((size_t)FUSED_BAR_WORDS));
        HIPCHK(hipMemsetAsync(m->fusedBar.p, 0, sizeof(unsigned int) * (size_t)FUSED_BAR_WORDS, s));
        m->fusedGen = 0;
    }
    if (++m->fusedGen == 0u) {
        HIPCHK(hipMemsetAsync(m->fusedBar.p, 0, sizeof(unsigned int) * BAR_LINE * (size_t)(RG + 64), s));
        m->fusedGen = 1u;
    }
    FusedArgs A;
    A.st = c->state.p; A.it = it;
    A.partial1 = c->partial.p; A.partial2 = c->partial.p + RG; A.partial3 = c->partial.p + 2 * RG;
    double *psi, *pA, *wA, *rA;
    MICHK(m->vecs({{WV_PSI, &psi}, {WV_PA, &pA}, {WV_WA, &wA}, {WV_RA, &rA}}));
    A.wA = wA; A.rD = m->rD.p; A.pA = pA; A.psi = psi; A.rA = rA; A.n = a->L.nCells;
    A.hist = m->hist.p; A.histLen = m->histLen;
    A.bar = m->fusedBar.p; A.gen = m->fusedGen;
    static const long long polls = (long long)sw::get(SW_PCG_FUSE_POLLS);
    A.maxPolls = polls;
    A.testMode = c->pcgFuseTest;
    void* args[1] = {&A};
    static const int coop = sw::get(SW_PCG_FUSE_COOP);
    if (coop) {
        if (hipLaunchCooperativeKernel(fn, dim3(RG), dim3(RB), args, (unsigned int)lds, s) != hipSuccess) {
            (void)hipGetLastError();
            c->pcgFuseRP = 0;
            return MI_ERR_UNSUPPORTED;
        }
    } else if (precond == MI_PRECOND_DIAGONAL) k_pcg_fused_r_p<1><<<RG, RB, lds, s>>>(A);
    else k_pcg_fused_r_p<2><<<RG, RB, lds, s>>>(A);
    if (precond == MI_PRECOND_DIAGONAL) k_pcg_fused_finish<1><<<RG, RB, 0, s>>>(A); else k_pcg_fused_finish<2><<<RG, RB, 0, s>>>(A);
    HIPCHK(hipGetLastError());
    c->stats[4] += 1;
    return MI_OK;
}

}
```

### rapidcfd-dev_amd/csrc/switches.hpp

```cpp
#pragma once
#include <cstdlib>

namespace mi {
#define MI_SWITCHES(X) \
    X(HOST_THREADS,            "MI_HOST_THREADS",            0,        ONCE,          USER,      nullptr,               "host threads of the one-time builds, clamped to 1..64; unset: the hardware's, divided by the launcher's local world size (host_parallel.hpp)") \
    X(HOST_THP,                "MI_HOST_THP",                1,        ONCE,          USER,      nullptr,               "host tables >= 4 MiB on 2 MiB boundaries, advised to transparent huge pages; a value that starts with 0: plain malloc (host_tables.hpp)") \
    X(PCG_PERSIST,             "MI_PCG_PERSIST",             1,        CTX,           USER,      "pcg_persist",         "0 never, 1 the persistent PCG kernel whenever the tiles fit the CUs' registers (persist.inc)") \
    X(WIN_DIRECT,              "MI_WIN_DIRECT",              1,        CTX,           USER,      "win_direct",          "tile operators of attached matrices read neighbour-rank values straight from the halo window (one launch for all tiles) instead of k_halo_pull + a second launch; 2 = also between processes that share a device") \
    X(PEER_POLLS,              "MI_PEER_POLLS",              20000000, ONCE,          USER,      nullptr,               "polls before a wait on a peer window gives up: several seconds (tests shorten it); read when the library loads (comm.inc: PEER_POLLS)") \
    X(GAMG_GRAPH,              "MI_GAMG_GRAPH",              1,        CTX,           USER,      nullptr,               "the V-cycle replays as a hipGraph; 0 = plain launches") \
    X(GAMG_GRAPH_ATTACHED,     "MI_GAMG_GRAPH_ATTACHED",     1,        CTX,           USER,      "gamg_graph_attached", "the V-cycle of a decomposed case replays as a hipGraph when every exchange of it is stream work (peer windows)") \
    X(TILE_REORDER,            "MI_TILE_REORDER",            -1,       ADDR,          USER,      nullptr,               "-1: Cuthill-McKee pre-ordering when the numbering has no locality, 0 never, 1 always (tiling.hpp)") \
    X(TILE_CELLS,              "MI_TILE_CELLS",              0,        ADDR,          USER,      nullptr,               "cells per tile; 0: 1024, coarse GAMG levels by MI_SMALL_TILES (engine.hip: addr_tile_params)") \
    X(TILE_SLOTS,              "MI_TILE_SLOTS",              4094,     ADDR,          USER,      nullptr,               "coefficient slots per tile") \
    \
    X(GAMG_FUSE,               "MI_GAMG_FUSE",               1,        CTX,           AB,        nullptr,               "fused transfers of the V-cycle (default cycle shape, single rank); 0 = the separate kernels") \
    X(FUSE_PROLOGUE,           "MI_FUSE_PROLOGUE",           1,        CTX,           AB,        "fuse_prologue",       "A psi, source - A psi and sumA in one pass over the coefficients, the prologue's sums batched; 0 = the separate passes, same bits") \
    X(PCG_FUSE_RP,             "MI_PCG_FUSE_RP",             1,        CTX,           AB,        "pcg_fuse_rp",         "residual update + next direction update as one launch (pcg_fused.inc); stored as 0 never, -1 once the device has been asked") \
    X(GAMG_INVERT_V2,          "MI_GAMG_INVERT_V2",          1,        CALL,          AB,        nullptr,               "the rewritten register-resident inversion kernel of the coarsest level; 0 = its first form, same bits") \
    X(MULTI_PIPE,              "MI_MULTI_PIPE",              1,        CTX,           AB,        nullptr,               "the multi-vector tile passes of the Krylov iterations as persistent pipelined workgroups (multi_pipe.inc): same bits, three-component PBiCG + DILU iteration 1 812 -> 1 643 us (profiles/r05_f_multi_pipe_ab.md)") \
    X(MULTI_TILE,              "MI_MULTI_TILE",              1,        CALL,          AB,        nullptr,               "multi-vector tile kernel for several right-hand sides; 0 = one single-vector launch each (multi.inc)") \
    X(PBICG_MULTI,             "MI_PBICG_MULTI",             1,        CALL,          AB,        nullptr,               "mi_pbicg_solve_multi runs its components as one multi-vector solve; 0 = one after the other (multi.inc)") \
    X(PBICG_PAIR,              "MI_PBICG_PAIR",              1,        CTX,           AB,        nullptr,               "PBiCG's A p / A^T pT (and the DILU pair) in one pass over the coefficients") \
    X(ROW16,                   "MI_ROW16",                   1,        ROWS,          AB,        nullptr,               "block-local 16-bit row tables of the assembly row passes (assembly.inc: R16)") \
    X(ENTRY16,                 "MI_ENTRY16",                 0,        ADDR,          AB,        nullptr,               "opt-in 16-bit row entries: half the entry bytes, measured 2-4 % slower (profiles/r01_n_compact_entries_ab.md)") \
    X(GAMG_DIRECT_SLOTS,       "MI_GAMG_DIRECT_SLOTS",       1,        HIER,          AB,        nullptr,               "direct agglomeration: slot-to-slot children lists between the levels' tile layouts") \
    X(GAMG_REG_INVERT,         "MI_GAMG_REG_INVERT",         1,        CALL,          AB,        nullptr,               "coarsest systems of up to 192 rows are inverted in registers") \
    X(GAMG_INVERT_OVERLAP,     "MI_GAMG_INVERT_OVERLAP",     1,        CALL,          AB,        nullptr,               "the coarsest-level inversion runs on the side stream beside the solve's prologue and first down-sweep") \
    X(GAMG_PIPELINE,           "MI_GAMG_PIPELINE",           1,        HIER,          AB,        nullptr,               "level layouts and transfer maps are built on other threads while the next level is matched") \
    X(GAMG_INHERIT_TILES,      "MI_GAMG_INHERIT_TILES",      0,        HIER,          AB,        nullptr,               "opt-in: a level takes its tiles from its fine side's tiles instead of clustering again (tiling.hpp: inherit_tiles); no gain measured") \
    X(GAMG_DEVICE_INVERT,      "MI_GAMG_DEVICE_INVERT",      -1,       CTX,           AB,        nullptr,               "inversion of the coarsest level: -1 by size, 0 on the host, 1 on the device") \
    X(PCG_DEFER_PSI,           "MI_PCG_DEFER_PSI",           1,        CTX,           AB,        nullptr,               "psi += alpha pA rides in the next k_pcg_update_p: one vector read less per iteration") \
    X(PCG_FUSE_FINAL,          "MI_PCG_FUSE_FINAL",          0,        CTX,           AB,        nullptr,               "convergence test fused into the next update_p; measured: no gain (332.0 vs 332.3 us/iter), kept as an option") \
    X(PCG_FUSE_COOP,           "MI_PCG_FUSE_COOP",           0,        ONCE,          AB,        nullptr,               "1: the fused PCG launch goes through hipLaunchCooperativeKernel -- ~22 us per launch on this runtime (pcg_fused.inc)") \
    X(FUSE_PERM,               "MI_FUSE_PERM",               1,        CTX,           AB,        nullptr,               "caller-order operators gather / scatter through e2c inside the tile kernel") \
    X(DPCG_FUSED,              "MI_DPCG_FUSED",              1,        CALL,          AB,        nullptr,               "distributed PCG with the halo exchange and the sums inside its kernels (peer.inc)") \
    X(PBICG_HOST_STEPPED,      "MI_PBICG_HOST_STEPPED",      0,        CTX,           AB,        nullptr,               "1: PBiCG / PBiCGStab through their host-stepped loops instead of the device-resident ones") \
    X(TILE_FLAGS,              "MI_TILE_FLAGS",              1,        CTX,           AB,        nullptr,               "bit0: coefficient segments are staged with non-temporal loads (read once per launch): Amul -4 % (profiles/r02_b_cache_policy_ab.md)") \
    X(TILE_PERSIST,            "MI_TILE_PERSIST",            0,        CTX,           AB,        nullptr,               "persistent tile launches: workgroups = resident slots, each walks a run of tiles") \
    X(XCD_ROWS,                "MI_XCD_ROWS",                1,        CTX,           AB,        nullptr,               "XCD-aware block mapping of the caller-order row passes") \
    X(SMALL_TILES,             "MI_SMALL_TILES",             1,        ADDR,          AB,        nullptr,               "coarse GAMG levels are cut into enough tiles for every CU, down to 128 cells (engine.hip: addr_tile_params)") \
    X(AMUL_BS,                 "MI_AMUL_BS",                 0,        CTX,           AB,        nullptr,               "threads per workgroup of the tile kernels: 256, 512 or 1024; anything else = 0 = chosen per launch from the LDS footprint") \
    X(PCG_BATCH,               "MI_PCG_BATCH",               16,       CTX,           AB,        nullptr,               "iterations per batch of the device-resident solver loops; below 1 = 1") \
    X(PCG_GRAPH,               "MI_PCG_GRAPH",               -1,       CTX,           AB,        nullptr,               "batches of PCG iterations replay as a hipGraph: -1 up to 4 M cells, 0 never, 1 always") \
    \
    X(PEER_HALO,               "MI_PEER_HALO",               1,        ATTACH,        TRANSPORT, nullptr,               "halo windows between the ranks when the communicator runs in peer mode") \
    X(PEER_FINEGRAINED,        "MI_PEER_FINEGRAINED",        1,        ATTACH | HIER, TRANSPORT, nullptr,               "peer windows in fine-grained device memory; 0 = ordinary device memory (coherent only between processes that share one device); HIER: the gather window of the coarsest level") \
    X(PEER_GLOBALIZE,          "MI_PEER_GLOBALIZE",          1,        CALL,          TRANSPORT, nullptr,               "a matrix's all-reduces go through the peer windows (peer.inc: peer_reduce_ready)") \
    X(PEER_ALLOW_COARSE,       "MI_PEER_ALLOW_COARSE",       0,        ATTACH | HIER, TRANSPORT, nullptr,               "accept windows in ordinary device memory although a peer is on another device (not coherent while a kernel polls); HIER: the gather window of the coarsest level") \
    X(GAMG_GATHER_WIN,         "MI_GAMG_GATHER_WIN",         1,        HIER,          TRANSPORT, nullptr,               "the coarsest level of a decomposed case is gathered through a peer window") \
    X(PERSIST_LITMUS,          "MI_PERSIST_LITMUS",          1,        PERSIST,       TRANSPORT, nullptr,               "grid-barrier litmus before a context's first persistent launch") \
    X(PERSIST_GRID,            "MI_PERSIST_GRID",            0,        CTX,           TRANSPORT, nullptr,               "workgroups of the persistent kernel; 0: one per CU") \
    X(PERSIST_SHARED,          "MI_PERSIST_SHARED",          0,        CTX,           TRANSPORT, nullptr,               "1 lets ranks that share a device use the persistent kernel -- tests only: their grids (MI_PERSIST_GRID) must fit the device TOGETHER") \
    X(PERSIST_ZP,              "MI_PERSIST_ZP",              1,        CALL,          TRANSPORT, nullptr,               "tiles per workgroup up to which the persistent PCG kernel publishes z = rD o rA and the second pA buffer (persist.inc, ZP)") \
    X(EVENT_ATTACH,            "MI_EVENT_ATTACH",            1,        CTX,           TRANSPORT, nullptr,               "0: plain hipEventRecord pairs around the Amul launch instead of kernel-attached events") \
    \
    X(PERSIST_SKIP_ARRIVAL,    "MI_PERSIST_SKIP_ARRIVAL",    0,        CALL,          DIAG,      nullptr,               "fault injection, n > 0: the last workgroup of the persistent kernel never arrives at its n-th barrier") \
    X(PERSIST_BAR_POLLS,       "MI_PERSIST_BAR_POLLS",       4000000,  CALL,          DIAG,      nullptr,               "polls before a grid-barrier wait gives up (persist.inc: BAR_POLLS, a few seconds); the fault tests shorten it") \
    X(PCG_FUSE_POLLS,          "MI_PCG_FUSE_POLLS",          1000,     ONCE,          DIAG,      nullptr,               "polls before a workgroup of the fused PCG launch leaves its barrier (pcg_fused.inc: FUSED_WAIT_POLLS)") \
    X(PCG_FUSE_TEST,           nullptr,                      0,        CTX,           DIAG,      "pcg_fuse_test",       "option only: workgroups of the fused launch that leave its barrier at once (pcg_fused.inc)") \
    X(ROW_CAP,                 "MI_ROW_CAP",                 0,        ROWS,          DIAG,      nullptr,               "forced staging capacity of the assembly row passes: a small value sends blocks down the unstaged path") \
    X(ROW_BS,                  "MI_ROW_BS",                  1024,     ROWS,          DIAG,      nullptr,               "cells per block of the one- and two-array row passes when the numbering is not tile-contiguous: 256, 512 or 1024") \
    X(GRAD_BS,                 "MI_GRAD_BS",                 256,      ROWS,          DIAG,      nullptr,               "... of the four-array gradient pass") \
    X(GAMG_ALWAYS_AGGLOMERATE, "MI_GAMG_ALWAYS_AGGLOMERATE", 0,        CTX,           DIAG,      nullptr,               "1: the level matrices are agglomerated again at every solve, also for unchanged coefficients") \
    X(MATCH_PARALLEL,          "MI_MATCH_PARALLEL",          0,        ADDR | HIER,   DIAG,      nullptr,               "1: large levels of the tile clustering (tiling.cpp) and of the pair agglomeration (gamg.cpp) are matched by the host threads; measured slower (profiles/r04_p_*)") \
    X(MATCH_LATER_ONLY,        "MI_MATCH_LATER_ONLY",        1,        HIER,          DIAG,      nullptr,               "the pair agglomeration looks only at faces to later cells (forward sweep over owned faces); 0 = every face of a cell") \
    X(DEBUG_MULTI,             "MI_DEBUG_MULTI",             0,        CALL,          DIAG,      nullptr,               "prints the multi-vector launches and their fall-backs to stderr") \
    X(DEBUG_PERSIST,           "MI_DEBUG_PERSIST",           0,        PERSIST,       DIAG,      nullptr,               "prints why persistent kernels were refused on a context to stderr")

enum Switch : int {
#define X(id, env, dflt, when, group, option, meaning) SW_##id,
    MI_SWITCHES(X)
#undef X
    SW_COUNT
};

inline int env_int(const char* name, int dflt)
{
    const char* v = name ? std::getenv(name) : nullptr;
    return (v && *v) ? std::atoi(v) : dflt;
}

namespace sw {
enum When : unsigned { ONCE = 1, CTX = 2, ADDR = 4, ROWS = 8, HIER = 16, ATTACH = 32, PERSIST = 64, CALL = 128 };
enum Group { USER, AB, TRANSPORT, DIAG };
struct Row { const char* env; int dflt; unsigned when; Group group; const char* option; };
constexpr Row table[SW_COUNT] = {
#define X(id, env, dflt, when, group, option, meaning) {env, dflt, when, group, option},
    MI_SWITCHES(X)
#undef X
};
inline int get(Switch s) { return env_int(table[s].env, table[s].dflt); }
inline const char* text(Switch s) { return table[s].env ? std::getenv(table[s].env) : nullptr; }
}
}
```

Baseline: 3774.

## Fold Amul tile partials in-kernel and drop fused-finish launch via stall recovery

The symmetric Amul kernel gets one extra workgroup that spin-waits on per-tile partial slots and reduces wA.pA itself, which removes the separate k_fold_partials launch. Separately, the k_pcg_fused_finish launch behind every fused r/p launch is dropped. A workgroup that times out on the grid barrier raises a stall word, and the host replays the finish and re-enqueues the remaining iterations at its next synchronisation point. This cuts two kernel launches per PCG iteration. The cost is polling workgroups, which risk deadlock if the extra block is scheduled before tiles finish, plus extra host checkpoint logic.

```diff
diff --git a/__graft_entry__.py b/__graft_entry__.py
--- a/__graft_entry__.py
+++ b/__graft_entry__.py
@@ -32,7 +32,7 @@
 def build() -> None:
     csrc = os.path.join(PKG_DIR, "csrc")
     srcs = [os.path.join(csrc, f) for f in ("engine.hip", "tiling.cpp", "gamg.cpp")]
-    deps = srcs + [os.path.join(csrc, f) for f in ("kernels.hip.hpp", "tiling.hpp", "host_parallel.hpp", "gamg.hpp", "gamg_engine.inc", "assembly.inc", "limited_grad.inc", "comm.inc", "peer.inc", "multi.inc", "multi_pipe.inc", "persist.inc", "pcg_fused.inc", "host_tables.hpp", "host_match.hpp", "switches.hpp")] + [os.path.join(ROOT, "include", "mi_ldu.h")]
+    deps = srcs + [os.path.join(csrc, f) for f in ("kernels.hip.hpp", "tiling.hpp", "host_parallel.hpp", "gamg.hpp", "gamg_engine.inc", "assembly.inc", "limited_grad.inc", "comm.inc", "peer.inc", "multi.inc", "multi_pipe.inc", "persist.inc", "pcg_fused.inc", "amul_fold.inc", "host_tables.hpp", "host_match.hpp", "switches.hpp")] + [os.path.join(ROOT, "include", "mi_ldu.h")]
     so = os.path.join(PKG_DIR, "librapidcfd_amd.so")
     if _stale(so, deps):
         hipcc = os.environ.get("HIPCC", "/opt/rocm/bin/hipcc")
diff --git a/include/mi_ldu.h b/include/mi_ldu.h
--- a/include/mi_ldu.h
+++ b/include/mi_ldu.h
@@ -59,6 +59,8 @@
 #define MI_STAT_PBICGSTAB_DEVICE 9
 #define MI_STAT_PBICGSTAB_HOST_STEPPED 10
 #define MI_STAT_PBICGSTAB_MID_EXIT 11
+#define MI_STAT_PCG_AMUL_FOLD 12
+#define MI_STAT_PCG_FUSED_FINISH 13
 int mi_ctx_stat(mi_ctx_t ctx, int32_t which, int64_t *out);
 const char *mi_last_error(void);
 int mi_device_available(void);
diff --git a/rapidcfd-dev_amd/csrc/amul_fold.inc b/rapidcfd-dev_amd/csrc/amul_fold.inc
--- /dev/null
+++ b/rapidcfd-dev_amd/csrc/amul_fold.inc
@@ -0,0 +1,67 @@
+namespace mi {
+
+constexpr unsigned long long FOLD_EMPTY = ~0ull;
+constexpr int FOLD_TERMS = 12;
+constexpr long long FOLD_POLLS = 400000;
+
+struct AmulFold {
+    const unsigned int* stall;
+    double* slots;
+    double* out;
+    int32_t* fault;
+};
+
+template <int BS, bool FOLD>
+__global__ __launch_bounds__(BS, BS >= 512 ? 8 : 1) void k_amul_fold(const TileArgs a, const AmulFold f)
+{
+    extern __shared__ __attribute__((aligned(16))) double smem[];
+    __shared__ double tilePartial;
+    {
+        const int32_t d = *a.done; const unsigned int s = *f.stall;
+        if (d != 0 || s != 0u) return;
+    }
+    const int b = blockIdx.x, nT = a.nPos, tid = threadIdx.x;
+    if (FOLD && b == nT) {
+        unsigned long long* slots = reinterpret_cast<unsigned long long*>(f.slots);
+        for (int t = tid; t < RG; t += BS) {
+            unsigned long long x[FOLD_TERMS];
+            bool all = true;
+            for (long long polls = 0;; ++polls) {
+#pragma unroll
+                for (int j = 0; j < FOLD_TERMS; ++j) {
+                    const int k = t + j * 1024;
+                    x[j] = k < nT ? __hip_atomic_load(slots + k, __ATOMIC_RELAXED, __HIP_MEMORY_SCOPE_AGENT) : 0ull;
+                }
+                all = true;
+#pragma unroll
+                for (int j = 0; j < FOLD_TERMS; ++j) all = all && x[j] != FOLD_EMPTY;
+                if (all || polls >= FOLD_POLLS) break;
+                __builtin_amdgcn_s_sleep(32);
+            }
+            if (!all) *f.fault = 1;
+            double v = 0.0;
+#pragma unroll
+            for (int j = 0; j < FOLD_TERMS; ++j)
+                if (t + j * 1024 < nT) v += __longlong_as_double((long long)x[j]);
+            f.out[t] = v;
+#pragma unroll
+            for (int j = 0; j < FOLD_TERMS; ++j)
+                if (t + j * 1024 < nT) __hip_atomic_store(slots + t + j * 1024, FOLD_EMPTY, __ATOMIC_RELAXED, __HIP_MEMORY_SCOPE_AGENT);
+        }
+        return;
+    }
+    const int per = nT >> 3;
+    const int p = (b < (per << 3)) ? (b & 7) * per + (b >> 3) : b;
+    if (!FOLD) { tile_body<OP_AMUL, false, false, BS, false>(a, p, smem); return; }
+    TileArgs a2 = a;
+    double* const mine = &tilePartial;
+    a2.dotPartial = mine - p;
+    tile_body<OP_AMUL, false, false, BS, false>(a2, p, smem);
+    if (tid == 0) {
+        unsigned long long bits = (unsigned long long)__double_as_longlong(tilePartial);
+        if (bits == FOLD_EMPTY) bits = 0x7FF8000000000000ull;
+        __hip_atomic_store(reinterpret_cast<unsigned long long*>(f.slots + p), bits, __ATOMIC_RELAXED, __HIP_MEMORY_SCOPE_AGENT);
+    }
+}
+
+}
diff --git a/rapidcfd-dev_amd/csrc/engine.hip b/rapidcfd-dev_amd/csrc/engine.hip
--- a/rapidcfd-dev_amd/csrc/engine.hip
+++ b/rapidcfd-dev_amd/csrc/engine.hip
@@ -4,6 +4,7 @@
 #include "tiling.hpp"
 #include "host_parallel.hpp"
 #include "switches.hpp"
+#include "amul_fold.inc"
 
 #include <algorithm>
 #include <atomic>
@@ -78,9 +79,9 @@
     int nCU = 0;
     bool keepSlotTables = false;
     int tileFlags = 0, attachEvents = 0, persist = 0, xcdRows = 0, deferPsi = 0, fusePerm = 0, pairAT = 0, fusePrologue = 0, multiPipe = 0, winDirect = 0, gamgGraphAttached = 0;
-    int pcgPersist = 0, pcgFuseRP = 0, pcgFuseTest = 0, persistGrid = 0, persistShared = 0, fuseFinal = 0, amulBS = 0, pcgBatch = 0, pcgGraph = 0, pbicgHostStepped = 0;
+    int pcgPersist = 0, pcgFuseRP = 0, pcgFuseTest = 0, pcgFoldAmul = 0, pcgLazyFinish = 0, persistGrid = 0, persistShared = 0, fuseFinal = 0, amulBS = 0, pcgBatch = 0, pcgGraph = 0, pbicgHostStepped = 0;
     int gamgDeviceInvert = 0, gamgAlwaysAgglomerate = 0, gamgGraph = 0, gamgFuse = 0;
-    int64_t stats[12] = {};
+    int64_t stats[14] = {};
     int persistCoop = -1;
     uint64_t faultEpoch = 0;
     struct mi_matrix_s* session = nullptr;
@@ -93,7 +94,7 @@
     {SW_TILE_FLAGS, &mi_ctx_s::tileFlags}, {SW_EVENT_ATTACH, &mi_ctx_s::attachEvents}, {SW_TILE_PERSIST, &mi_ctx_s::persist}, {SW_XCD_ROWS, &mi_ctx_s::xcdRows},
     {SW_PCG_DEFER_PSI, &mi_ctx_s::deferPsi}, {SW_FUSE_PERM, &mi_ctx_s::fusePerm}, {SW_PBICG_PAIR, &mi_ctx_s::pairAT}, {SW_FUSE_PROLOGUE, &mi_ctx_s::fusePrologue},
     {SW_MULTI_PIPE, &mi_ctx_s::multiPipe}, {SW_WIN_DIRECT, &mi_ctx_s::winDirect}, {SW_GAMG_GRAPH_ATTACHED, &mi_ctx_s::gamgGraphAttached}, {SW_PCG_PERSIST, &mi_ctx_s::pcgPersist},
-    {SW_PCG_FUSE_RP, &mi_ctx_s::pcgFuseRP}, {SW_PCG_FUSE_TEST, &mi_ctx_s::pcgFuseTest}, {SW_PERSIST_GRID, &mi_ctx_s::persistGrid}, {SW_PERSIST_SHARED, &mi_ctx_s::persistShared},
+    {SW_PCG_FUSE_RP, &mi_ctx_s::pcgFuseRP}, {SW_PCG_FUSE_TEST, &mi_ctx_s::pcgFuseTest}, {SW_PCG_FOLD_AMUL, &mi_ctx_s::pcgFoldAmul}, {SW_PCG_LAZY_FINISH, &mi_ctx_s::pcgLazyFinish}, {SW_PERSIST_GRID, &mi_ctx_s::persistGrid}, {SW_PERSIST_SHARED, &mi_ctx_s::persistShared},
     {SW_PCG_FUSE_FINAL, &mi_ctx_s::fuseFinal}, {SW_AMUL_BS, &mi_ctx_s::amulBS}, {SW_PCG_BATCH, &mi_ctx_s::pcgBatch}, {SW_PCG_GRAPH, &mi_ctx_s::pcgGraph},
     {SW_PBICG_HOST_STEPPED, &mi_ctx_s::pbicgHostStepped}, {SW_GAMG_DEVICE_INVERT, &mi_ctx_s::gamgDeviceInvert}, {SW_GAMG_ALWAYS_AGGLOMERATE, &mi_ctx_s::gamgAlwaysAgglomerate},
     {SW_GAMG_GRAPH, &mi_ctx_s::gamgGraph}, {SW_GAMG_FUSE, &mi_ctx_s::gamgFuse},
@@ -176,6 +177,12 @@
     bool pcgPReady = false;
     DevBuf<unsigned int> fusedBar;
     unsigned int fusedGen = 0;
+    unsigned int* fusedStallHost = nullptr;
+    bool fusedUnchecked = false;
+    int fusedEnd = 0, fusedPrecond = MI_PRECOND_DIAGONAL;
+    DevBuf<unsigned int> amulGateZero;
+    DevBuf<double> amulFoldSlots;
+    AmulFold amulFold = {nullptr, nullptr, nullptr, nullptr};
     Table<hipEvent_t> evPool;
     hipGraphExec_t pcgGraph = nullptr;
     struct { int precond = -1, batch = 0, histLen = 0; const void* hist = nullptr; const void* psi = nullptr; } pcgGraphKey;
@@ -766,6 +773,24 @@
 
 namespace {
 
+template <int BS, bool FOLD>
+int launch_amul_fold(mi_matrix_s* m, const TileArgs& args, int nTiles, size_t lds)
+{
+    mi_ctx_s* cx = m->addr->ctx;
+    hipStream_t s = cx->stream;
+    const void* fn = (const void*)k_amul_fold<BS, FOLD>;
+    if (!cx->ldsAttrSet.count(fn)) {
+        HIPCHK(hipFuncSetAttribute(fn, hipFuncAttributeMaxDynamicSharedMemorySize, 159 * 1024));
+        cx->ldsAttrSet.insert(fn);
+    }
+    const int grid = nTiles + (FOLD ? 1 : 0);
+    if (m->kevStart) hipExtLaunchKernelGGL((k_amul_fold<BS, FOLD>), dim3(grid), dim3(BS), (uint32_t)lds, s, m->kevStart, m->kevStop, 0, args, m->amulFold);
+    else k_amul_fold<BS, FOLD><<<grid, BS, lds, s>>>(args, m->amulFold);
+    HIPCHK(hipGetLastError());
+    if (FOLD) cx->stats[12] += 1;
+    return MI_OK;
+}
+
 template <int OP, bool ASYM, bool TRANS, bool C16>
 int launch_tile_bs(mi_matrix_s* m, const TileArgs& args, int nTiles, size_t lds)
 {
@@ -773,6 +798,13 @@
     int bs = m->addr->ctx->amulBS;
     if (bs == 0) bs = (lds > 53 * 1024) ? 1024 : (m->addr->L.maxCells <= 256 ? 256 : 512);
     if (nTiles <= 0) return MI_OK;
+    if constexpr (OP == OP_AMUL && !ASYM && !TRANS && !C16)
+        if (m->amulFold.stall) {
+            const bool fold = m->amulFold.slots != nullptr;
+            if (bs == 1024) return fold ? launch_amul_fold<1024, true>(m, args, nTiles, lds) : launch_amul_fold<1024, false>(m, args, nTiles, lds);
+            if (bs == 512) return fold ? launch_amul_fold<512, true>(m, args, nTiles, lds) : launch_amul_fold<512, false>(m, args, nTiles, lds);
+            return fold ? launch_amul_fold<256, true>(m, args, nTiles, lds) : launch_amul_fold<256, false>(m, args, nTiles, lds);
+        }
 #define MI_LAUNCH(BS)                                                                                                   \
     {                                                                                                                   \
         mi_ctx_s* cx = m->addr->ctx;                                                                                    \
@@ -1427,7 +1459,7 @@
     HIPCHK(hipStreamSynchronize(c->stream));
     if (c->hostState->fault) {
         c->faultEpoch++;
-        return fail(MI_ERR_DEVICE, "persistent PCG kernel: a workgroup never reached a grid barrier (ran out of polls); the results of this solve are not valid");
+        return fail(MI_ERR_DEVICE, "a device-side wait ran out of polls (persistent PCG kernel: a workgroup never reached a grid barrier; folding Amul: a tile's partial never arrived); the results of this solve are not valid");
     }
     return MI_OK;
 }
@@ -1518,8 +1550,18 @@
     return MI_OK;
 }
 
+bool pcg_amul_gated_usable(const mi_matrix_s* m)
+{
+    const mi_addr_s* a = m->addr;
+    return !comm_attached(m) && !m->asym && !a->compact && !a->ctx->persist && a->L.nTiles > 0;
+}
 bool pcg_fused_rp_usable(const mi_matrix_s* m, int precond);
 int pcg_fused_rp_launch(mi_matrix_s* m, int it, int precond);
+bool pcg_fused_lazy(const mi_matrix_s* m);
+int pcg_fused_words(mi_matrix_s* m);
+unsigned int* pcg_fused_stall_word(mi_matrix_s* m);
+int pcg_fused_checkpoint(mi_matrix_s* m, bool* recovered = nullptr);
+int pcg_fused_forget(mi_matrix_s* m);
 bool pcg_persist_usable(const mi_matrix_s* m, int precond);
 int pcg_persist_enqueue(mi_matrix_s* m, int n_iters, int precond);
 int pcg_enqueue(mi_matrix_s* m, int it0, int count, int precond, int evStride)
@@ -1540,6 +1582,22 @@
     GateDone gate(m);
     bool fusedRP = it0 >= 0 && pcg_fused_rp_usable(m, precond);
     if (it0 < 0) m->pcgPReady = false;
+    const bool gatedAmul = it0 >= 0 && precond != MI_PRECOND_AINV && pcg_amul_gated_usable(m);
+    const bool foldAmul = gatedAmul && c->pcgFoldAmul != 0 && a->L.nTiles <= FOLD_TERMS * 1024;
+    const bool lazy = fusedRP && gatedAmul && pcg_fused_lazy(m);
+    if (m->fusedUnchecked && !lazy) {
+        HIPCHK(hipStreamSynchronize(s));
+        MICHK(pcg_fused_checkpoint(m));
+    }
+    if ((foldAmul || lazy) && m->amulGateZero.n == 0) {
+        MICHK(m->amulGateZero.alloc(1));
+        HIPCHK(hipMemsetAsync(m->amulGateZero.p, 0, sizeof(unsigned int), s));
+    }
+    if (foldAmul && m->amulFoldSlots.n != (size_t)a->L.nTiles) {
+        MICHK(m->amulFoldSlots.alloc((size_t)a->L.nTiles));
+        HIPCHK(hipMemsetAsync(m->amulFoldSlots.p, 0xFF, sizeof(double) * (size_t)a->L.nTiles, s));
+    }
+    if (lazy) { MICHK(pcg_fused_words(m)); m->fusedEnd = it0 + count; m->fusedPrecond = precond; }
     for (int k = 0; k < count; ++k) {
         const int it = it0 < 0 ? -1 : it0 + k;
         if (m->pcgPReady) {
@@ -1561,11 +1619,13 @@
             if (c->attachEvents) { m->kevStart = m->evPool[ev]; m->kevStop = m->evPool[ev + 1]; }
             else HIPCHK(hipEventRecord(m->evPool[ev], s));
         }
+        if (foldAmul || (lazy && fusedRP))
+            m->amulFold = AmulFold{(lazy && fusedRP) ? pcg_fused_stall_word(m) : m->amulGateZero.p, foldAmul ? m->amulFoldSlots.p : nullptr, P2, &c->state.p->fault};
         const int rcA = tile_op<OP_AMUL>(m, false, pA, nullptr, nullptr, wA, 0.0, m->tilePartial.p);
-        m->kevStart = nullptr; m->kevStop = nullptr;
+        m->kevStart = nullptr; m->kevStop = nullptr; m->amulFold.stall = nullptr;
         MICHK(rcA);
         if (rec && !c->attachEvents) HIPCHK(hipEventRecord(m->evPool[ev + 1], s));
-        k_fold_partials<<<1, 1024, 0, s>>>(m->tilePartial.p, a->L.nTiles, P2);
+        if (!foldAmul) k_fold_partials<<<1, 1024, 0, s>>>(m->tilePartial.p, a->L.nTiles, P2);
         MICHK(globalize(m, P2));
         m->pcgPReady = false;
         if (fusedRP) {
@@ -1623,6 +1683,7 @@
         return fail(MI_ERR_STATE, "mi_pcg_begin: another matrix has a PCG session open on this context (one session per context: it owns the solver scratch)");
     mi_addr_s* a = m->addr;
     HIPCHK(hipSetDevice(a->ctx->device));
+    MICHK(pcg_fused_forget(m));
     PcgVecs v;
     MICHK(stage_in(m, v, psi0, source));
     MICHK(solve_prologue(m, ctl, v.psi, v.src, v.wA, v.rA, history_len));
@@ -1656,6 +1717,7 @@
     m->pcgIt += n_iters;
     if (amul_ms_sum) {
         HIPCHK(hipStreamSynchronize(m->addr->ctx->stream));
+        MICHK(pcg_fused_checkpoint(m));
         const int ns = (n_iters + stride - 1) / stride;
         float tot = 0;
         for (int i = 0; i < ns; ++i) { float ms = 0; HIPCHK(hipEventElapsedTime(&ms, m->evPool[(size_t)2 * i], m->evPool[(size_t)2 * i + 1])); tot += ms; }
@@ -1671,6 +1733,10 @@
     HIPCHK(hipSetDevice(a->ctx->device));
     double* psi;
     MICHK(m->vec(WV_PSI, &psi));
+    if (m->fusedUnchecked) {
+        HIPCHK(hipStreamSynchronize(a->ctx->stream));
+        MICHK(pcg_fused_checkpoint(m));
+    }
     MICHK(pcg_flush(m));
     if (psi_out) k_scatter_perm<<<RG, RB, 0, a->ctx->stream>>>(psi, a->perm(), psi_out, a->L.nCells);
     HIPCHK(hipGetLastError());
@@ -1720,7 +1786,9 @@
         }
         return mi_pcg_end(m, psi, perf, hist_host, hist_len);
     }
-    MICHK(drive_batches(m, ctl, m->pcgIt, 2, [m](int nb) { return mi_pcg_iterate(m, nb, nullptr); }));
+    MICHK(drive_batches(m, ctl, m->pcgIt, 2, [m](int nb) { return mi_pcg_iterate(m, nb, nullptr); },
+                        [m, c]() -> int { MICHK(fetch_state(c)); bool again = false; MICHK(pcg_fused_checkpoint(m, &again)); return again ? fetch_state(c) : MI_OK; },
+                        [c] { return c->hostState->done != 0; }));
     return mi_pcg_end(m, psi, perf, hist_host, hist_len);
 }
 
@@ -2200,6 +2268,8 @@
     HIPCHK(hipEventRecord(c->ev1, c->stream));
     HIPCHK(hipEventSynchronize(c->ev1));
     HIPCHK(hipEventElapsedTime(ms_out, c->ev0, c->ev1));
+    HIPCHK(hipStreamSynchronize(c->stream));
+    MICHK(pcg_fused_checkpoint(m));
     m->pcgActive = false; c->session = nullptr;
     if (amul_ms_out) { float t = 0; MICHK(mi_bench_amul(m, iters, &t)); *amul_ms_out = t; }
     return MI_OK;
@@ -2291,6 +2361,7 @@
 {
     if (pcgGraph) (void)hipGraphExecDestroy(pcgGraph);
     if (mhostState) (void)hipHostFree(mhostState);
+    if (fusedStallHost) (void)hipHostFree(fusedStallHost);
     for (auto* w : work) delete w;
     for (auto e : evPool) (void)hipEventDestroy(e);
     if (dpc) {
diff --git a/rapidcfd-dev_amd/csrc/pcg_fused.inc b/rapidcfd-dev_amd/csrc/pcg_fused.inc
--- a/rapidcfd-dev_amd/csrc/pcg_fused.inc
+++ b/rapidcfd-dev_amd/csrc/pcg_fused.inc
@@ -5,6 +5,8 @@
 constexpr int FUSED_LP = 2544;
 constexpr int FUSED_BAR_WORDS = BAR_LINE * (RG + 64) + RG + 64;
 constexpr int FUSED_PEND_AT = BAR_LINE * (RG + 64);
+constexpr int FUSED_STALL_AT = FUSED_PEND_AT + RG + 1;
+static_assert(FUSED_STALL_AT < FUSED_BAR_WORDS, "the stall word lies inside the barrier array");
 constexpr long long FUSED_WAIT_POLLS = 1000;
 static_assert(sw::table[SW_PCG_FUSE_POLLS].dflt == FUSED_WAIT_POLLS, "switches.hpp: the default of MI_PCG_FUSE_POLLS is FUSED_WAIT_POLLS");
 
@@ -20,6 +22,7 @@
     unsigned int* bar; unsigned int gen;
     long long maxPolls;
     int testMode;
+    unsigned int *stall, *stallHost;
 };
 
 __device__ __forceinline__ void st_agent(double* p, double v)
@@ -112,14 +115,18 @@
     __shared__ double red[RB / 64];
     __shared__ int flag;
     PcgState* __restrict__ st = a.st;
-    if (st->done) return;
     const int it = a.it;
     const unsigned int b = blockIdx.x, tid = threadIdx.x;
     const bool lead = b == 0 && tid == 0;
+    if (st->done) { if (lead && a.stall && st->rItP1 >= it) st->pApplyItP1 = it; return; }
+    if (a.stall) {
+        const unsigned int w = __hip_atomic_load(a.stall, __ATOMIC_RELAXED, __HIP_MEMORY_SCOPE_AGENT);
+        if (w != 0u && w != (unsigned int)it + 1u) return;
+    }
     const double wApA = sum_partials(a.partial2, red);
     if (fabs(wApA) / st->normFactor < SP_VSMALL) {
         if (tid == 0) a.partial3[b] = -1.0;
-        if (lead) { st->singular = 1; st->done = 1; }
+        if (lead) { st->singular = 1; st->done = 1; if (a.stall && st->rItP1 >= it) st->pApplyItP1 = it; }
         return;
     }
     const double wArAold = st->wArA[it & 1];
@@ -179,6 +186,10 @@
     if (!fused_wait(a.bar, a.gen, a.maxPolls, a.testMode, &flag)) {
         if (tid == 0) __hip_atomic_store(&a.bar[FUSED_PEND_AT + b], 1u, __ATOMIC_RELAXED, __HIP_MEMORY_SCOPE_AGENT);
         if (lead) __hip_atomic_store(&a.bar[FUSED_PEND_AT + RG], 1u, __ATOMIC_RELAXED, __HIP_MEMORY_SCOPE_AGENT);
+        if (tid == 0 && a.stall) {
+            __hip_atomic_store(a.stall, (unsigned int)it + 1u, __ATOMIC_RELAXED, __HIP_MEMORY_SCOPE_AGENT);
+            __hip_atomic_store(a.stallHost, (unsigned int)it + 1u, __ATOMIC_RELAXED, __HIP_MEMORY_SCOPE_SYSTEM);
+        }
         return;
     }
     const FusedScalars sc = fused_scalars<true>(st, it, a.partial3, a.partial1, wArAold, red);
@@ -269,6 +280,44 @@
     return c->pcgFuseRP != 0 && !comm_attached(m) && (precond == MI_PRECOND_DIAGONAL || precond == MI_PRECOND_NONE) && !c->fuseFinal;
 }
 
+bool pcg_fused_lazy(const mi_matrix_s* m) { return m->addr->ctx->pcgLazyFinish != 0 && pcg_amul_gated_usable(m); }
+unsigned int* pcg_fused_stall_word(mi_matrix_s* m) { return m->fusedBar.p + FUSED_STALL_AT; }
+
+int pcg_fused_words(mi_matrix_s* m)
+{
+    hipStream_t s = m->addr->ctx->stream;
+    if (m->fusedBar.n < (size_t)FUSED_BAR_WORDS) {
+        MICHK(m->fusedBar.alloc((size_t)FUSED_BAR_WORDS));
+        HIPCHK(hipMemsetAsync(m->fusedBar.p, 0, sizeof(unsigned int) * (size_t)FUSED_BAR_WORDS, s));
+        m->fusedGen = 0;
+    }
+    if (!m->fusedStallHost) {
+        HIPCHK(hipHostMalloc((void**)&m->fusedStallHost, sizeof(unsigned int)));
+        *m->fusedStallHost = 0u;
+    }
+    return MI_OK;
+}
+
+int pcg_fused_args(mi_matrix_s* m, int it, FusedArgs& A)
+{
+    mi_addr_s* a = m->addr;
+    mi_ctx_s* c = a->ctx;
+    A.st = c->state.p; A.it = it;
+    A.partial1 = c->partial.p; A.partial2 = c->partial.p + RG; A.partial3 = c->partial.p + 2 * RG;
+    double *psi, *pA, *wA, *rA;
+    MICHK(m->vecs({{WV_PSI, &psi}, {WV_PA, &pA}, {WV_WA, &wA}, {WV_RA, &rA}}));
+    A.wA = wA; A.rD = m->rD.p; A.pA = pA; A.psi = psi; A.rA = rA; A.n = a->L.nCells;
+    A.hist = m->hist.p; A.histLen = m->histLen;
+    A.bar = m->fusedBar.p; A.gen = m->fusedGen;
+    static const long long polls = (long long)sw::get(SW_PCG_FUSE_POLLS);
+    A.maxPolls = polls;
+    A.testMode = c->pcgFuseTest;
+    const bool lazy = pcg_fused_lazy(m);
+    A.stall = lazy ? m->fusedBar.p + FUSED_STALL_AT : nullptr;
+    A.stallHost = lazy ? m->fusedStallHost : nullptr;
+    return MI_OK;
+}
+
 int pcg_fused_rp_launch(mi_matrix_s* m, int it, int precond)
 {
     mi_addr_s* a = m->addr;
@@ -287,26 +336,13 @@
         c->pcgFuseRP = ((int64_t)perCU * nCU >= RG) ? 1 : 0;
         if (!c->pcgFuseRP) return MI_ERR_UNSUPPORTED;
     }
-    if (m->fusedBar.n < (size_t)FUSED_BAR_WORDS) {
-        MICHK(m->fusedBar.alloc((size_t)FUSED_BAR_WORDS));
-        HIPCHK(hipMemsetAsync(m->fusedBar.p, 0, sizeof(unsigned int) * (size_t)FUSED_BAR_WORDS, s));
-        m->fusedGen = 0;
-    }
+    MICHK(pcg_fused_words(m));
     if (++m->fusedGen == 0u) {
         HIPCHK(hipMemsetAsync(m->fusedBar.p, 0, sizeof(unsigned int) * BAR_LINE * (size_t)(RG + 64), s));
         m->fusedGen = 1u;
     }
     FusedArgs A;
-    A.st = c->state.p; A.it = it;
-    A.partial1 = c->partial.p; A.partial2 = c->partial.p + RG; A.partial3 = c->partial.p + 2 * RG;
-    double *psi, *pA, *wA, *rA;
-    MICHK(m->vecs({{WV_PSI, &psi}, {WV_PA, &pA}, {WV_WA, &wA}, {WV_RA, &rA}}));
-    A.wA = wA; A.rD = m->rD.p; A.pA = pA; A.psi = psi; A.rA = rA; A.n = a->L.nCells;
-    A.hist = m->hist.p; A.histLen = m->histLen;
-    A.bar = m->fusedBar.p; A.gen = m->fusedGen;
-    static const long long polls = (long long)sw::get(SW_PCG_FUSE_POLLS);
-    A.maxPolls = polls;
-    A.testMode = c->pcgFuseTest;
+    MICHK(pcg_fused_args(m, it, A));
     void* args[1] = {&A};
     static const int coop = sw::get(SW_PCG_FUSE_COOP);
     if (coop) {
@@ -317,10 +353,53 @@
         }
     } else if (precond == MI_PRECOND_DIAGONAL) k_pcg_fused_r_p<1><<<RG, RB, lds, s>>>(A);
     else k_pcg_fused_r_p<2><<<RG, RB, lds, s>>>(A);
-    if (precond == MI_PRECOND_DIAGONAL) k_pcg_fused_finish<1><<<RG, RB, 0, s>>>(A); else k_pcg_fused_finish<2><<<RG, RB, 0, s>>>(A);
+    if (A.stall) m->fusedUnchecked = true;
+    else {
+        if (precond == MI_PRECOND_DIAGONAL) k_pcg_fused_finish<1><<<RG, RB, 0, s>>>(A); else k_pcg_fused_finish<2><<<RG, RB, 0, s>>>(A);
+        c->stats[13] += 1;
+    }
     HIPCHK(hipGetLastError());
     c->stats[4] += 1;
     return MI_OK;
 }
 
-}
+int pcg_fused_checkpoint(mi_matrix_s* m, bool* recovered)
+{
+    if (recovered) *recovered = false;
+    if (!m->fusedUnchecked) return MI_OK;
+    m->fusedUnchecked = false;
+    mi_ctx_s* c = m->addr->ctx;
+    hipStream_t s = c->stream;
+    while (*m->fusedStallHost != 0u) {
+        const int stalled = (int)*m->fusedStallHost - 1;
+        *m->fusedStallHost = 0u;
+        if (recovered) *recovered = true;
+        FusedArgs A;
+        MICHK(pcg_fused_args(m, stalled, A));
+        const int precond = m->fusedPrecond, end = m->fusedEnd;
+        if (precond == MI_PRECOND_DIAGONAL) k_pcg_fused_finish<1><<<RG, RB, 0, s>>>(A); else k_pcg_fused_finish<2><<<RG, RB, 0, s>>>(A);
+        HIPCHK(hipGetLastError());
+        c->stats[13] += 1;
+        HIPCHK(hipMemsetAsync(m->fusedBar.p + FUSED_STALL_AT, 0, sizeof(unsigned int), s));
+        if (stalled + 1 < end) {
+            m->pcgPReady = true;
+            MICHK(pcg_enqueue(m, stalled + 1, end - (stalled + 1), precond, 0));
+        }
+        m->fusedUnchecked = false;
+        HIPCHK(hipStreamSynchronize(s));
+    }
+    return MI_OK;
+}
+
+int pcg_fused_forget(mi_matrix_s* m)
+{
+    if (!m->fusedUnchecked) return MI_OK;
+    m->fusedUnchecked = false;
+    hipStream_t s = m->addr->ctx->stream;
+    HIPCHK(hipStreamSynchronize(s));
+    *m->fusedStallHost = 0u;
+    HIPCHK(hipMemsetAsync(m->fusedBar.p + FUSED_PEND_AT, 0, sizeof(unsigned int) * (size_t)(RG + 64), s));
+    return MI_OK;
+}
+
+}
diff --git a/rapidcfd-dev_amd/csrc/switches.hpp b/rapidcfd-dev_amd/csrc/switches.hpp
--- a/rapidcfd-dev_amd/csrc/switches.hpp
+++ b/rapidcfd-dev_amd/csrc/switches.hpp
@@ -17,6 +17,8 @@
     X(GAMG_FUSE,               "MI_GAMG_FUSE",               1,        CTX,           AB,        nullptr,               "fused transfers of the V-cycle (default cycle shape, single rank); 0 = the separate kernels") \
     X(FUSE_PROLOGUE,           "MI_FUSE_PROLOGUE",           1,        CTX,           AB,        "fuse_prologue",       "A psi, source - A psi and sumA in one pass over the coefficients, the prologue's sums batched; 0 = the separate passes, same bits") \
     X(PCG_FUSE_RP,             "MI_PCG_FUSE_RP",             1,        CTX,           AB,        "pcg_fuse_rp",         "residual update + next direction update as one launch (pcg_fused.inc); stored as 0 never, -1 once the device has been asked") \
+    X(PCG_FOLD_AMUL,           "MI_PCG_FOLD_AMUL",           1,        CTX,           AB,        nullptr,               "single-GPU PCG: the symmetric Amul folds its own per-tile partials of wA.pA, one extra workgroup (amul_fold.inc); 0 = the k_fold_partials launch behind it, same bits") \
+    X(PCG_LAZY_FINISH,         "MI_PCG_LAZY_FINISH",         1,        CTX,           AB,        nullptr,               "no k_pcg_fused_finish launch behind the fused PCG launch: a workgroup that leaves raises a stall word, the host recovers where it waits anyway (pcg_fused.inc); 0 = the launch behind every fused launch, same bits") \
     X(GAMG_INVERT_V2,          "MI_GAMG_INVERT_V2",          1,        CALL,          AB,        nullptr,               "the rewritten register-resident inversion kernel of the coarsest level; 0 = its first form, same bits") \
     X(MULTI_PIPE,              "MI_MULTI_PIPE",              1,        CTX,           AB,        nullptr,               "the multi-vector tile passes of the Krylov iterations as persistent pipelined workgroups (multi_pipe.inc): same bits, three-component PBiCG + DILU iteration 1 812 -> 1 643 us (profiles/r05_f_multi_pipe_ab.md)") \
     X(MULTI_TILE,              "MI_MULTI_TILE",              1,        CALL,          AB,        nullptr,               "multi-vector tile kernel for several right-hand sides; 0 = one single-vector launch each (multi.inc)") \
```

Result: no change. 3819, median of 6 (+1.2%).
